# Project-MONAI/MONAI

Hardware: AMD Instinct MI355X
Metric: voxels/s sliding-window 3D seg (512^3 vol, 96^3 win, ov 0.5) at 1/8 GPU (higher is better)
Workload: dtype f32; 1 GPU; BasicUNet 5-class seed 1, 512^3 CT phantom in HBM, 96^3 win ov 0.5 gaussian, sw_batch 4 (engine: <= 64 windows per launch); parallelism=1 GPU

## Files before the change

### include/monai_amd.h

```cpp
#ifndef MONAI_AMD_H
#define MONAI_AMD_H

#include <stddef.h>
#include <stdint.h>

#ifdef __cplusplus
extern "C" {
#endif

#define MH_OK 0
#define MH_ERR_ARG (-1)
#define MH_ERR_LAUNCH (-2)
#define MH_ERR_UNSUPPORTED (-3)

typedef struct mh_tensor5 {
    float* data;
    int64_t n_stride;
    const float* nrm;
    int64_t nrm_n_stride;
    int32_t N, C, D, H, W;
} mh_tensor5;

int mh_version(void);
const char* mh_last_error(void);



int mh_window_extract_f32(const float* vol, int C, int D, int H, int W, const int32_t* sz, int nz,
                          const int32_t* sy, int ny, const int32_t* sx, int nx, int w0, int nwin, int rd, int rh,
                          int rw, float* out, void* stream);

int mh_sw_blend_f32(const float* logits, int64_t window_stride, const float* imp, float* out, int K, int D, int H, int W,
                    int rd, int rh, int rw, const int32_t* sz, int nz, const int32_t* sy, int ny, const int32_t* sx,
                    int nx, int premultiplied, void* stream);

int mh_sw_blend_buffered_f32(const float* logits, int64_t window_stride, const float* imp, float* out, int K, int D, int H, int W, int rd, int rh, int rw,
                             const int32_t* sz, int nz, const int32_t* sy, int ny, const int32_t* sx, int nx, int buffer_axis, int buffer_steps, int premultiplied, void* stream);

int mh_sw_mosaic_class_counts(int n, int log2m, int32_t* counts5);
int mh_sw_blend_mosaic_f32(const float* logits, const int64_t* class_base, int log2m_z, int log2m_y, int log2m_x, const float* imp, int imp_factored, float* out, int K,
                           int D, int H, int W, int rd, int rh, int rw, const int32_t* sz, int nz, const int32_t* sy, int ny, const int32_t* sx, int nx,
                           void* stream);

int mh_sw_blend_argmax_f32(const float* logits, int64_t window_stride, const float* imp, void* labels, int labels_u8, int K, int D,
                           int H, int W, int rd, int rh, int rw, const int32_t* sz, int nz, const int32_t* sy, int ny,
                           const int32_t* sx, int nx, int premultiplied, void* stream);

int mh_patch_accumulate_f32(float* values, uint8_t* counts, const float* patch, int NC, int D, int H, int W, int pd, int ph,
                            int pw, int z0, int y0, int x0, void* stream);
int mh_patch_accumulate_batch_f32(float* values, uint8_t* counts, const float* patches, int npatch, const int32_t* loc, int NC, int D, int H, int W,
                                  int pd, int ph, int pw, void* stream);
int mh_avg_finalize_f32(float* values, const uint8_t* counts, int64_t n, void* stream);


#define MH_ALGO_AUTO 0
#define MH_ALGO_DIRECT 1
#define MH_ALGO_WINO2D 2
#define MH_ALGO_H2 3
#define MH_ALGO_FP32 4
int mh_conv3d_k3_select(int algo, int input_bounded, int Cin, int Cout, int D, int H, int W);
int mh_conv3d_k3_num_configs(void);
int mh_conv3d_k3_h2_config(void);
int mh_conv3d_k3_h2c_config(void);
int mh_conv3d_k3_c1_config(void);
int mh_conv3d_k3_h2v_config(void);
int mh_conv3d_k3_h2w_config(void);
int mh_conv3d_k3_h2w_fits(int D, int H, int W);
int mh_conv3d_k3_accepts(int cfg, int Cin, int Cout);
int64_t mh_conv3d_k3_packed_floats(int cfg, int Cin, int Cout);
int mh_conv3d_k3_pack_f32(int cfg, const float* w, int Cin, int Cout, float* packed, void* stream);
int mh_conv3d_k3_stat_tiles(int cfg, int D, int H, int W);
int mh_conv3d_k3_f32(int cfg, const mh_tensor5* in, const float* packed_w, const float* bias,
                     const mh_tensor5* out, float* stats, void* stream);
int mh_conv3d_k3_pool_accepts(int cfg, int Cin, int Cout, int D, int H, int W);
int mh_conv3d_k3_pool_f32(int cfg, const mh_tensor5* in, const float* packed_w, const float* bias, const mh_tensor5* out, float* stats, float* pool_max, float* pool_min,
                          int64_t pool_n_stride, void* stream);
int mh_pool_select_f32(float* pool_max, const float* pool_min, const float* nrm, int64_t nrm_n_stride, int N, int C, int64_t n_stride, int64_t vol, void* stream);
int mh_conv3d_k3_accumulate_f32(int cfg, const mh_tensor5* in, const float* packed_w, const float* bias, const mh_tensor5* out, float* stats, void* stream);

int mh_instnorm_stat_tiles(int D, int H, int W);
int mh_instnorm_stats_f32(const mh_tensor5* x, float* stats, void* stream);
int mh_instnorm_finalize_f32(const float* stats, int tiles, int N, int C, const float* gamma, const float* beta,
                             float eps, float slope, float* nrm, int64_t nrm_n_stride, void* stream);
int mh_groupnorm_finalize_f32(const float* stats, int tiles, int N, int C, int groups, const float* gamma, const float* beta, float eps,
                              float slope, float* nrm, int64_t nrm_n_stride, void* stream);

int mh_nrm_identity_f32(float* nrm, int N, int C, int64_t nrm_n_stride, void* stream);

int mh_maxpool2_f32(const mh_tensor5* in, const mh_tensor5* out, void* stream);

int mh_deconv_k2s2_f32(const mh_tensor5* in, const float* w, const float* bias, const mh_tensor5* out,
                       void* stream);

int mh_deconv_k2s2_h2_accepts(int Cin, int Cout, int D, int H, int W);
int64_t mh_deconv_k2s2_h2_packed_floats(int Cin, int Cout);
int mh_deconv_k2s2_h2_pack_f32(const float* w, int Cin, int Cout, float* packed, void* stream);
int mh_deconv_k2s2_h2_f32(const mh_tensor5* in, const float* packed, const float* bias, const mh_tensor5* out, void* stream);

int mh_upconv_k4s2_accepts(int Cin, int Cout, int Dl, int Hl, int Wl);
int64_t mh_upconv_k4s2_packed_floats(int Cin, int Cout);
int mh_upconv_k4s2_pack_f32(const float* w4, int Cin, int Cout, float* packed, void* stream);
int mh_upconv_k4s2_stat_tiles(int Dl, int Hl, int Wl);
int mh_upconv_k4s2_f32(const mh_tensor5* low, const float* packed, const float* bias_table, const mh_tensor5* out, int accumulate, float* stats, void* stream);

int mh_conv3d_k3s2_accepts(int Cin, int Cout, int D, int H, int W);
int64_t mh_conv3d_k3s2_packed_floats(int Cin, int Cout);
int64_t mh_conv3d_k3s2_workspace_floats(int N, int Cin, int D, int H, int W);
int mh_conv3d_k3s2_stat_tiles(int D, int H, int W);
int mh_conv3d_k3s2_pack_f32(const float* w, int Cin, int Cout, float* packed, void* stream);
int mh_conv3d_k3s2_f32(const mh_tensor5* in, const float* packed, const float* bias, const mh_tensor5* out, float* workspace, float* stats, int fused, void* stream);

int mh_conv1x1_f32(const mh_tensor5* in, const float* w, const float* bias, const mh_tensor5* out,
                   void* stream);
int mh_conv1x1_stat_tiles(int D, int H, int W);
int mh_conv1x1_stats_f32(const mh_tensor5* in, const float* w, const float* bias, const mh_tensor5* out, float* stats, void* stream);

int mh_conv1x1_h2_accepts(int Cin, int Cout, int D, int H, int W);
int64_t mh_conv1x1_h2_packed_floats(int Cin, int Cout);
int mh_conv1x1_h2_pack_f32(const float* w, int Cout, int Cin, float* packed, void* stream);
int mh_conv1x1_h2_f32(const mh_tensor5* in, const float* packed, const float* bias, const mh_tensor5* out, float* stats, void* stream);

int mh_conv1x1_windows_f32(const mh_tensor5* in, const float* w, const float* bias, float* base, int Cout, const int64_t* place, void* stream);


int mh_add_act_f32(const mh_tensor5* a, const mh_tensor5* b, float slope, const mh_tensor5* out, void* stream);

int mh_conv1x1_sum2_accepts(int Cout, int D, int H, int W);
int mh_conv1x1_sum2_f32(const mh_tensor5* a, const mh_tensor5* b, float slope, const float* w, const float* bias, const mh_tensor5* out, void* stream);

int mh_pad_replicate_f32(const mh_tensor5* in, const mh_tensor5* out, void* stream);

int mh_pixelshuffle_f32(const mh_tensor5* in, const mh_tensor5* out, int fz, int pad_pool, void* stream);

int mh_attention_f32(const float* qkv, float* out, int B, int S, int heads, int head_dim, float scale, void* stream);

int mh_window_attention_f32(const float* qkv, const float* bias_t, const float* mask, float* out, int BW, int nW, int S, int heads,
                            int head_dim, float scale, int exact_fp32, void* stream);

int mh_window_attention_rel_accepts(int S, int head_dim, int table_rows);
int mh_window_attention_rel_f32(const float* qkv, const float* rel_table, int table_rows, const int32_t* coord, int coord_off, const int32_t* region,
                                float* out, int BW, int nW, int S, int heads, int head_dim, float scale, void* stream);

int64_t mh_linear_packed_floats(int N, int K);
int mh_linear_pack_f32(const float* w, int N, int K, float* packed, void* stream);
int mh_linear_f32(const float* x, const float* packed_w, const float* bias, const float* residual, float* y, int64_t M, int N, int K, int act,
                  void* stream);
int mh_linear_tile_f32(const float* x, const float* packed_w, const float* bias, const float* residual, float* y, int64_t M, int N, int K, int act,
                       int tile, void* stream);

int mh_layernorm_f32(const float* x, const float* gamma, const float* beta, float eps, float* y, int64_t M, int K, void* stream);

int mh_layernorm_gather_accepts(int K);
int mh_layernorm_gather_f32(const float* x, const float* gamma, const float* beta, float eps, float* y, int64_t M_out, int K, const int32_t* src_row, void* stream);
int mh_linear_scatter_f32(const float* x, const float* packed_w, const float* bias, const float* residual, float* y, int64_t M, int N, int K, int act,
                          const int32_t* dst_row, void* stream);


int mh_conv3d_k3_strided_f32(const mh_tensor5* in, const float* packed_w, const float* bias, const mh_tensor5* out,
                             int stride, void* stream);
int mh_conv3d_k3_strided3_f32(const mh_tensor5* in, const float* packed_w, const float* bias, const mh_tensor5* out, int sz, int sy, int sx,
                              void* stream);
int mh_deconv_ks_f32(const mh_tensor5* in, const float* w, const float* bias, const mh_tensor5* out, int fz, int fy, int fx, void* stream);

int mh_deconv_k3_f32(const mh_tensor5* in, const float* w, const float* bias, const mh_tensor5* out, int stride,
                     void* stream);


int64_t mh_affine_resample_workspace_bytes(int Do, int Ho, int Wo);
int mh_affine_resample_f32(const float* src, int NC, int Di, int Hi, int Wi, float* dst, int Do, int Ho, int Wo,
                           const double* m, int mode, int pad, int align_corners, int compute_f64, void* workspace,
                           void* stream);

int mh_grid_resample_f32(const float* src, int NC, int Di, int Hi, int Wi, const void* coords, int coords_f64,
                         const double* scale3, const double* offset3, float* dst, int Do, int Ho, int Wo, int mode,
                         int pad, int align_corners, int compute_f64, void* stream);

int mh_grid_pull(const void* src, const void* grid, void* out, int is_f64, int B, int C, int X, int Y, int Z, int Xo,
                 int Yo, int Zo, const int32_t* bound3, const int32_t* interp3, int extrapolate, void* stream);

int mh_pushpull(const void* source, const void* grid, const void* target, void* out, void* grad, int is_f64, int ndim, int B,
                int C, int X, int Y, int Z, int Xo, int Yo, int Zo, const int32_t* bound3, const int32_t* interp3,
                int extrapolate, int do_pull, int do_push, int do_count, int do_grad, int do_sgrad, int target_k, void* stream);


int mh_pointwise_f32(int op, const float* src, float* dst, int64_t n, float param, void* stream);
int mh_channel_reduce_f32(int op, const float* src, float* dst, int C, int64_t n, void* stream);
int mh_onehot_f32(const float* labels, float* dst, int K, int64_t n, void* stream);


int mh_scale_intensity_range_f32(const float* src, float* dst, int64_t n, float a_min, float a_div, int rescale, float b_scale, float b_min,
                                 int clip_lo, float lo, int clip_hi, float hi, void* stream);
int mh_foreground_bbox_workspace_ints(int D, int H);
int mh_foreground_bbox_f32(const float* src, int C, int D, int H, int W, int32_t* workspace, int32_t* box6, void* stream);
int mh_crop_pad_f32(const float* src, float* dst, int C, int D, int H, int W, int Do, int Ho, int Wo, int sz, int sy, int sx, float value,
                    void* stream);

int64_t mh_normalize_stats_workspace_doubles(int C, int64_t n);
int mh_normalize_stats_f32(const float* src, int C, int64_t n, int nonzero, double* workspace, float* subdiv, void* stream);
int mh_normalize_apply_f32(const float* src, float* dst, int C, int64_t n, int nonzero, const float* subdiv, void* stream);
int64_t mh_minmax_workspace_floats(int C, int64_t n);
int mh_minmax_f32(const float* src, int C, int64_t n, float* workspace, float* table, void* stream);
int mh_minmax_scale_f32(const float* src, float* dst, int C, int64_t n, const float* table, int rescale, float b_scale, float b_min,
                        int flat_has_mul, float flat_mul, void* stream);
int mh_flip_permute_f32(const float* src, float* dst, int C, const int32_t* in_size3, const int32_t* perm3, const int32_t* flip3, void* stream);


int mh_separable_filter3d_f32(const float* src, float* dst, int NC, int D, int H, int W, const float* kz, int kz_n,
                              const float* ky, int ky_n, const float* kx, int kx_n, void* stream);

#ifdef __cplusplus
}
#endif
#endif
```

### monai_amd/_lib.py

```python

from __future__ import annotations

import ctypes as C
import os
from typing import Optional, Sequence

import torch

from ._fallback import UnsupportedOnDevice

_HERE = os.path.dirname(os.path.abspath(__file__))
LIB_PATH = os.environ.get("MONAI_AMD_LIB") or os.path.join(_HERE, "csrc", "libmonai_amd.so")


class MhTensor5(C.Structure):

    _fields_ = [
        ("data", C.c_void_p),
        ("n_stride", C.c_int64),
        ("nrm", C.c_void_p),
        ("nrm_n_stride", C.c_int64),
        ("N", C.c_int32),
        ("C", C.c_int32),
        ("D", C.c_int32),
        ("H", C.c_int32),
        ("W", C.c_int32),
    ]


_I, _L, _P, _F = C.c_int, C.c_int64, C.c_void_p, C.c_float
_T = C.POINTER(MhTensor5)
_IA = C.POINTER(C.c_int32)

SIGNATURES = {
    "mh_version": (_I, []),
    "mh_last_error": (C.c_char_p, []),
    "mh_window_extract_f32": (_I, [_P, _I, _I, _I, _I, _IA, _I, _IA, _I, _IA, _I, _I, _I, _I, _I, _I, _P, _P]),
    "mh_patch_accumulate_f32": (_I, [_P, _P, _P] + [_I] * 10 + [_P]),
    "mh_patch_accumulate_batch_f32": (_I, [_P, _P, _P, _I, _IA] + [_I] * 7 + [_P]),
    "mh_avg_finalize_f32": (_I, [_P, _P, C.c_int64, _P]),
    "mh_pointwise_f32": (_I, [_I, _P, _P, _L, _F, _P]),
    "mh_channel_reduce_f32": (_I, [_I, _P, _P, _I, _L, _P]),
    "mh_onehot_f32": (_I, [_P, _P, _I, _L, _P]),
    "mh_scale_intensity_range_f32": (_I, [_P, _P, _L, _F, _F, _I, _F, _F, _I, _F, _I, _F, _P]),
    "mh_foreground_bbox_workspace_ints": (_I, [_I, _I]),
    "mh_foreground_bbox_f32": (_I, [_P, _I, _I, _I, _I, _P, _P, _P]),
    "mh_crop_pad_f32": (_I, [_P, _P] + [_I] * 10 + [_F, _P]),
    "mh_sw_blend_f32": (_I, [_P, _L, _P, _P, _I, _I, _I, _I, _I, _I, _I, _IA, _I, _IA, _I, _IA, _I, _I, _P]),
    "mh_sw_blend_buffered_f32": (_I, [_P, _L, _P, _P, _I, _I, _I, _I, _I, _I, _I, _IA, _I, _IA, _I, _IA, _I, _I, _I, _I, _P]),
    "mh_sw_mosaic_class_counts": (_I, [_I, _I, _IA]),
    "mh_sw_blend_mosaic_f32": (_I, [_P, C.POINTER(C.c_int64), _I, _I, _I, _P, _I, _P, _I, _I, _I, _I, _I, _I, _I, _IA, _I, _IA, _I, _IA, _I, _P]),
    "mh_sw_blend_argmax_f32": (_I, [_P, _L, _P, _P, _I, _I, _I, _I, _I, _I, _I, _I, _IA, _I, _IA, _I, _IA, _I, _I, _P]),
    "mh_conv3d_k3_select": (_I, [_I, _I, _I, _I, _I, _I, _I]),
    "mh_conv3d_k3_h2_config": (_I, []),
    "mh_conv3d_k3_h2c_config": (_I, []),
    "mh_conv3d_k3_c1_config": (_I, []),
    "mh_conv3d_k3_h2v_config": (_I, []),
    "mh_conv3d_k3_h2w_config": (_I, []),
    "mh_conv3d_k3_h2w_fits": (_I, [_I, _I, _I]),
    "mh_conv3d_k3_num_configs": (_I, []),
    "mh_conv3d_k3_accepts": (_I, [_I, _I, _I]),
    "mh_conv3d_k3_packed_floats": (_L, [_I, _I, _I]),
    "mh_conv3d_k3_pack_f32": (_I, [_I, _P, _I, _I, _P, _P]),
    "mh_conv3d_k3_stat_tiles": (_I, [_I, _I, _I, _I]),
    "mh_conv3d_k3_f32": (_I, [_I, _T, _P, _P, _T, _P, _P]),
    "mh_conv3d_k3_accumulate_f32": (_I, [_I, _T, _P, _P, _T, _P, _P]),
    "mh_conv3d_k3_pool_accepts": (_I, [_I, _I, _I, _I, _I, _I]),
    "mh_conv3d_k3_pool_f32": (_I, [_I, _T, _P, _P, _T, _P, _P, _P, _L, _P]),
    "mh_pool_select_f32": (_I, [_P, _P, _P, _L, _I, _I, _L, _L, _P]),
    "mh_instnorm_stat_tiles": (_I, [_I, _I, _I]),
    "mh_instnorm_stats_f32": (_I, [_T, _P, _P]),
    "mh_instnorm_finalize_f32": (_I, [_P, _I, _I, _I, _P, _P, _F, _F, _P, _L, _P]),
    "mh_groupnorm_finalize_f32": (_I, [_P, _I, _I, _I, _I, _P, _P, _F, _F, _P, _L, _P]),
    "mh_flip_permute_f32": (_I, [_P, _P, _I, _IA, _IA, _IA, _P]),
    "mh_normalize_stats_workspace_doubles": (_L, [_I, _L]),
    "mh_normalize_stats_f32": (_I, [_P, _I, _L, _I, _P, _P, _P]),
    "mh_normalize_apply_f32": (_I, [_P, _P, _I, _L, _I, _P, _P]),
    "mh_minmax_workspace_floats": (_L, [_I, _L]),
    "mh_minmax_f32": (_I, [_P, _I, _L, _P, _P, _P]),
    "mh_minmax_scale_f32": (_I, [_P, _P, _I, _L, _P, _I, _F, _F, _I, _F, _P]),
    "mh_nrm_identity_f32": (_I, [_P, _I, _I, _L, _P]),
    "mh_maxpool2_f32": (_I, [_T, _T, _P]),
    "mh_deconv_k2s2_f32": (_I, [_T, _P, _P, _T, _P]),
    "mh_upconv_k4s2_accepts": (_I, [_I, _I, _I, _I, _I]),
    "mh_upconv_k4s2_packed_floats": (_L, [_I, _I]),
    "mh_upconv_k4s2_pack_f32": (_I, [_P, _I, _I, _P, _P]),
    "mh_upconv_k4s2_stat_tiles": (_I, [_I, _I, _I]),
    "mh_upconv_k4s2_f32": (_I, [_T, _P, _P, _T, _I, _P, _P]),
    "mh_deconv_k2s2_h2_accepts": (_I, [_I, _I, _I, _I, _I]),
    "mh_deconv_k2s2_h2_packed_floats": (_L, [_I, _I]),
    "mh_deconv_k2s2_h2_pack_f32": (_I, [_P, _I, _I, _P, _P]),
    "mh_deconv_k2s2_h2_f32": (_I, [_T, _P, _P, _T, _P]),
    "mh_conv3d_k3s2_accepts": (_I, [_I, _I, _I, _I, _I]),
    "mh_conv3d_k3s2_packed_floats": (_L, [_I, _I]),
    "mh_conv3d_k3s2_workspace_floats": (_L, [_I, _I, _I, _I, _I]),
    "mh_conv3d_k3s2_stat_tiles": (_I, [_I, _I, _I]),
    "mh_conv3d_k3s2_pack_f32": (_I, [_P, _I, _I, _P, _P]),
    "mh_conv3d_k3s2_f32": (_I, [_T, _P, _P, _T, _P, _P, _I, _P]),
    "mh_conv1x1_f32": (_I, [_T, _P, _P, _T, _P]),
    "mh_conv1x1_stat_tiles": (_I, [_I, _I, _I]),
    "mh_conv1x1_stats_f32": (_I, [_T, _P, _P, _T, _P, _P]),
    "mh_conv1x1_h2_accepts": (_I, [_I, _I, _I, _I, _I]),
    "mh_conv1x1_h2_packed_floats": (_L, [_I, _I]),
    "mh_conv1x1_h2_pack_f32": (_I, [_P, _I, _I, _P, _P]),
    "mh_conv1x1_h2_f32": (_I, [_T, _P, _P, _T, _P, _P]),
    "mh_conv1x1_sum2_accepts": (_I, [_I, _I, _I, _I]),
    "mh_conv1x1_sum2_f32": (_I, [_T, _T, _F, _P, _P, _T, _P]),
    "mh_conv1x1_windows_f32": (_I, [_T, _P, _P, _P, _I, C.POINTER(C.c_int64), _P]),
    "mh_conv3d_k3_strided_f32": (_I, [_T, _P, _P, _T, _I, _P]),
    "mh_conv3d_k3_strided3_f32": (_I, [_T, _P, _P, _T, _I, _I, _I, _P]),
    "mh_deconv_ks_f32": (_I, [_T, _P, _P, _T, _I, _I, _I, _P]),
    "mh_deconv_k3_f32": (_I, [_T, _P, _P, _T, _I, _P]),
    "mh_add_act_f32": (_I, [_T, _T, _F, _T, _P]),
    "mh_pad_replicate_f32": (_I, [_T, _T, _P]),
    "mh_pixelshuffle_f32": (_I, [_T, _T, _I, _I, _P]),
    "mh_attention_f32": (_I, [_P, _P, _I, _I, _I, _I, _F, _P]),
    "mh_window_attention_f32": (_I, [_P, _P, _P, _P, _I, _I, _I, _I, _I, _F, _I, _P]),
    "mh_window_attention_rel_accepts": (_I, [_I, _I, _I]),
    "mh_window_attention_rel_f32": (_I, [_P, _P, _I, _P, _I, _P, _P, _I, _I, _I, _I, _I, _F, _P]),
    "mh_linear_packed_floats": (_L, [_I, _I]),
    "mh_linear_pack_f32": (_I, [_P, _I, _I, _P, _P]),
    "mh_linear_f32": (_I, [_P, _P, _P, _P, _P, _L, _I, _I, _I, _P]),
    "mh_linear_tile_f32": (_I, [_P, _P, _P, _P, _P, _L, _I, _I, _I, _I, _P]),
    "mh_layernorm_f32": (_I, [_P, _P, _P, _F, _P, _L, _I, _P]),
    "mh_layernorm_gather_accepts": (_I, [_I]),
    "mh_layernorm_gather_f32": (_I, [_P, _P, _P, _F, _P, _L, _I, _P, _P]),
    "mh_linear_scatter_f32": (_I, [_P, _P, _P, _P, _P, _L, _I, _I, _I, _P, _P]),
    "mh_affine_resample_workspace_bytes": (_L, [_I, _I, _I]),
    "mh_affine_resample_f32": (_I, [_P, _I, _I, _I, _I, _P, _I, _I, _I, C.POINTER(C.c_double), _I, _I, _I, _I, _P, _P]),
    "mh_separable_filter3d_f32": (_I, [_P, _P, _I, _I, _I, _I, C.POINTER(C.c_float), _I, C.POINTER(C.c_float), _I, C.POINTER(C.c_float), _I, _P]),
    "mh_grid_pull": (_I, [_P, _P, _P, _I, _I, _I, _I, _I, _I, _I, _I, _I, _IA, _IA, _I, _P]),
    "mh_pushpull": (_I, [_P, _P, _P, _P, _P] + [_I] * 10 + [_IA, _IA] + [_I] * 7 + [_P]),
    "mh_grid_resample_f32": (_I, [_P, _I, _I, _I, _I, _P, _I, C.POINTER(C.c_double), C.POINTER(C.c_double), _P, _I, _I, _I, _I, _I, _I, _I, _P]),
}


class KernelRejected(RuntimeError):
    """An entry point declined a VALID call it has no kernel for (MH_ERR_UNSUPPORTED: a size / shape rule) without launching: callers with an alternative
    path catch THIS, not RuntimeError.  Bad arguments (MH_ERR_ARG: null pointers, mismatched shapes, misalignment -- caller bugs), launch failures and HIP
    errors stay plain RuntimeErrors and must surface."""


class Library:

    def __init__(self, path: str):
        if not os.path.exists(path):
            raise RuntimeError(
                f"monai_amd: HIP extension not built ({path} missing). Run `python -m monai_amd.build` "
                "(hipcc --offload-arch=gfx950); there is no CPU fallback."
            )
        self.path = path
        self._dll = C.CDLL(path)
        for name, (res, args) in SIGNATURES.items():
            fn = getattr(self._dll, name)
            fn.restype, fn.argtypes = res, args
            setattr(self, "_" + name, fn)

    def last_error(self) -> str:
        return self._mh_last_error().decode("utf-8", "replace")

    def check(self, rc: int) -> None:
        if rc == -3:
            raise KernelRejected(f"monai_amd: {self.last_error()} (code {rc})")
        if rc != 0:
            raise RuntimeError(f"monai_amd: {self.last_error()} (code {rc})")

    def call(self, name: str, *args) -> None:
        self.check(getattr(self, "_" + name)(*args))

    def query(self, name: str, *args) -> int:
        rc = getattr(self, "_" + name)(*args)
        if rc < 0:
            raise RuntimeError(f"monai_amd: {self.last_error()} (code {rc})")
        return int(rc)


_LIB: Optional[Library] = None


def lib() -> Library:
    global _LIB
    if _LIB is None:
        _LIB = Library(LIB_PATH)
    return _LIB


def require_device(*tensors: torch.Tensor, dtypes=(torch.float32,)) -> None:
    for t in tensors:
        if t is None:
            continue
        if not t.is_cuda:
            raise UnsupportedOnDevice(
                "monai_amd: this path runs only on an MI355X (ROCm) device tensor; got a CPU tensor. "
                "There is no CPU fallback in the product path."
            )
        if t.dtype not in dtypes:
            raise UnsupportedOnDevice(f"monai_amd: dtype {t.dtype} is not accepted on this path (expected one of {dtypes})")


def stream_ptr(t: torch.Tensor) -> C.c_void_p:
    if t.is_cuda:
        return C.c_void_p(torch.cuda.current_stream(t.device).cuda_stream)
    return C.c_void_p(0)


def ptr(t: Optional[torch.Tensor]) -> C.c_void_p:
    return C.c_void_p(0 if t is None else t.data_ptr())


def int_array(values: Sequence[int]):
    return (C.c_int32 * len(values))(*[int(v) for v in values])


def tensor5(t: torch.Tensor, nrm: Optional[torch.Tensor] = None) -> MhTensor5:
    if t.dim() != 5:
        raise RuntimeError(f"monai_amd: expected a 5-D NCDHW tensor, got shape {tuple(t.shape)}")
    n, c, d, h, w = t.shape
    st = t.stride()
    if st[4] != 1 or st[3] != w or st[2] != h * w or st[1] != d * h * w:
# ... 12 lines not shown
```

### monai_amd/config.py

```python
import os

HAS_EXT = True
USE_COMPILED = HAS_EXT and os.getenv("BUILD_MONAI", "0") == "1"


CONV_ALGOS = {"auto": 0, "direct": 1, "wino2d": 2, "h2": 3, "fp32": 4}
CONV_ALGO = None


def conv_algo() -> int:
    name = CONV_ALGO if CONV_ALGO is not None else os.environ.get("MONAI_AMD_CONV_ALGO", "auto")
    try:
        return CONV_ALGOS[str(name).lower()]
    except KeyError:
        raise ValueError(f"monai_amd: unknown convolution family {name!r} (one of {sorted(CONV_ALGOS)})") from None


class conv_algo_scope:

    def __init__(self, name: str):
        if str(name).lower() not in CONV_ALGOS:
            raise ValueError(f"monai_amd: unknown convolution family {name!r} (one of {sorted(CONV_ALGOS)})")
        self.name = str(name).lower()

    def __enter__(self):
        global CONV_ALGO
        self._saved, CONV_ALGO = CONV_ALGO, self.name
        return self

    def __exit__(self, *exc):
        global CONV_ALGO
        CONV_ALGO = self._saved
        return False


UPCAT_FUSED = None


def upcat_fused() -> bool:
    v = UPCAT_FUSED if UPCAT_FUSED is not None else os.environ.get("MONAI_AMD_UPCAT_FUSED", "1")
    return str(v).lower() not in ("0", "false", "off", "no")


UPCAT_ORDER = None


def upcat_order() -> str:
    v = str(UPCAT_ORDER if UPCAT_ORDER is not None else os.environ.get("MONAI_AMD_UPCAT_ORDER", "conv_first")).lower()
    if v not in ("conv_first", "term_first"):
        raise ValueError(f"monai_amd: unknown UpCat order {v!r} (conv_first or term_first)")
    return v


CONV_HALVES = None


def conv_halves() -> bool:
    v = CONV_HALVES if CONV_HALVES is not None else os.environ.get("MONAI_AMD_CONV_HALVES", "1")
    return str(v).lower() not in ("0", "false", "off", "no")


RESIDUAL_ACC = None


def residual_accumulate() -> bool:
    v = RESIDUAL_ACC if RESIDUAL_ACC is not None else os.environ.get("MONAI_AMD_RESIDUAL_ACC", "1")
    return str(v).lower() not in ("0", "false", "off", "no")


POOL_FUSED = None


def pool_fused() -> bool:
    v = POOL_FUSED if POOL_FUSED is not None else os.environ.get("MONAI_AMD_POOL_FUSED", "1")
    return str(v).lower() not in ("0", "false", "off", "no")


STRIDED_H2 = None


def strided_h2() -> bool:
    v = STRIDED_H2 if STRIDED_H2 is not None else os.environ.get("MONAI_AMD_STRIDED_H2", "1")
    return str(v).lower() not in ("0", "false", "off", "no") and conv_algo() in (CONV_ALGOS["auto"], CONV_ALGOS["h2"])


STRIDED_H2_FUSED = None


def strided_h2_fused() -> str:
    v = str(STRIDED_H2_FUSED if STRIDED_H2_FUSED is not None else os.environ.get("MONAI_AMD_STRIDED_H2_FUSED", "auto")).lower()
    return "0" if v in ("0", "false", "off", "no") else ("1" if v in ("1", "true", "on", "yes") else "auto")


SMALL_VOLUME_H2 = None


def small_volume_h2() -> bool:
    v = SMALL_VOLUME_H2 if SMALL_VOLUME_H2 is not None else os.environ.get("MONAI_AMD_SMALL_VOLUME_H2", "1")
    return str(v).lower() not in ("0", "false", "off", "no")


DECONV_H2 = None


def deconv_h2() -> bool:
    v = DECONV_H2 if DECONV_H2 is not None else os.environ.get("MONAI_AMD_DECONV_H2", "1")
    return str(v).lower() not in ("0", "false", "off", "no") and conv_algo() in (CONV_ALGOS["auto"], CONV_ALGOS["h2"])


SWIN_FUSED_MOVES = None


def swin_fused_moves() -> bool:
    v = SWIN_FUSED_MOVES if SWIN_FUSED_MOVES is not None else os.environ.get("MONAI_AMD_SWIN_FUSED_MOVES", "1")
    return str(v).lower() not in ("0", "false", "off", "no")


SWIN_REL_ATTENTION = None


def swin_rel_attention() -> bool:
    v = SWIN_REL_ATTENTION if SWIN_REL_ATTENTION is not None else os.environ.get("MONAI_AMD_SWIN_REL_ATTENTION", "1")
    return str(v).lower() not in ("0", "false", "off", "no")
```

### monai_amd/csrc/capi.hip

```cpp
#include <hip/hip_runtime.h>

#include <stdarg.h>
#include <stdio.h>
#include <stdlib.h>
#include <string.h>

#include "kernels/common.h"
#include "kernels/attention.h"
#include "kernels/conv3d_mfma.h"
#include "kernels/conv3d_wino2p.h"
#include "kernels/conv3d_h2.h"
#include "kernels/conv3d_wino_h2.h"
#include "kernels/upconv_h2.h"
#include "kernels/conv3d_s2_h2.h"
#include "kernels/deconv_h2.h"
#include "kernels/conv3d_vol_h2.h"
#include "kernels/conv3d_c1.h"
#include "kernels/dense.h"
#include "kernels/gaussian.h"
#include "kernels/grid_pull.h"
#include "kernels/pushpull.h"
#include "kernels/post.h"
#include "kernels/preproc.h"
#include "kernels/nn_simple.h"
// ... 433 lines not shown
static inline int hw_blocks(int D, int H, int W) { return hw_regions(H, W) * cdiv(D, hw_zchunk(D, H, W)); }

int mh_conv3d_k3_num_configs(void) { return MH_CFG_WINO2D; }
int mh_conv3d_k3_h2_config(void) { return MH_CFG_H2; }
int mh_conv3d_k3_h2c_config(void) { return MH_CFG_H2C; }
int mh_conv3d_k3_c1_config(void) { return MH_CFG_C1; }
int mh_conv3d_k3_h2v_config(void) { return MH_CFG_H2V; }
int mh_conv3d_k3_h2w_config(void) { return MH_CFG_H2W; }
int mh_conv3d_k3_h2w_fits(int D, int H, int W) { return hw_fits(D, H, W) ? 1 : 0; }

int mh_conv3d_k3_pool_accepts(int cfg, int Cin, int Cout, int D, int H, int W) {
    if (cfg == MH_CFG_H2W) return Cin == HWG_CIN && Cout >= HWG_CN && Cout % HWG_CN == 0 && D % 2 == 0 && hw_fits(D, H, W);
    if (cfg != MH_CFG_H2 || D < 2 || H < 2 || W < 2 || D % 2 || H % 2 || W % 4) return 0;
    if (!(Cin >= H2_KC && Cin % H2_KC == 0 && Cin <= H2_NRM_MAX && Cout >= H2_CN && Cout % (H2_CN / 2) == 0) || !h2_fits(D, H, W)) return 0;
    return !h2_wide(H, W) && h2_zchunk(D, H, W) % 2 == 0;
}
int mh_conv3d_k3_accepts(int cfg, int Cin, int Cout) {
    if (cfg == 0) return 1;
    if (cfg == MH_CFG_WINO2D) return Cin >= 8 && Cin % 8 == 0 && Cout >= W2_CN && Cout % W2_CN == 0;
    if (cfg == MH_CFG_H2) return Cin >= H2_KC && Cin % H2_KC == 0 && Cin <= H2_NRM_MAX && Cout >= H2_CN && Cout % (H2_CN / 2) == 0;
    if (cfg == MH_CFG_H2C) return Cin >= H2_KC && Cin % H2_KC == 0 && Cin <= H2_NRM_MAX && Cout >= 16 && Cout % 16 == 0;
    if (cfg == MH_CFG_C1) return Cin == 1 && Cout >= 8 && Cout % 8 == 0;
    if (cfg == MH_CFG_H2V) return Cin >= 16 && Cin % 16 == 0 && Cin <= HV_CIN_MAX && Cout >= 32 && Cout % 32 == 0;
    if (cfg == MH_CFG_H2W) return Cin == HWG_CIN && Cout >= HWG_CN && Cout % HWG_CN == 0;
    if (cfg < 0 || cfg > MH_NUM_CFG) return 0;
    return Cout >= 1 && cin_padded(cfg, Cin) <= Cfg1::NRM_MAX;
}

int mh_conv3d_k3_select(int algo, int input_bounded, int Cin, int Cout, int D, int H, int W) {
    if (Cin < 1 || Cout < 1 || D < 1 || H < 1 || W < 1) return fail(MH_ERR_ARG, "conv3d_k3_select: bad argument");
    if (algo < MH_ALGO_AUTO || algo > MH_ALGO_FP32) return fail(MH_ERR_ARG, "conv3d_k3_select: unknown algorithm family %d", algo);
    int best = 0;
    double best_score = 0.0;
    for (int c = 1; c <= MH_NUM_CFG; ++c) {
        const CfgInfo& k = kCfg[c];
        if (!mh_conv3d_k3_accepts(c, Cin, Cout)) continue;
        const double util = (double)D * H * W / ((double)cdiv(D, k.tz) * k.tz * cdiv(H, k.ty) * k.ty * cdiv(W, k.tx) * k.tx);
        const double cpad = ((double)Cin / cin_padded(c, Cin)) * ((double)Cout / cout_padded(c, Cout));
        const double score = util * cpad * (1.0 + 0.02 * (k.cn / 32)) * kPref[c];
        if (score > best_score) { best_score = score; best = c; }
    }
    if (mh_conv3d_k3_accepts(MH_CFG_WINO2D, Cin, Cout) && H % 2 == 0 && W % 8 == 0) {
        const bool big = H % W2_B == 0 && W % W2_B == 0 && D >= 48 && H >= 48 && W >= 48;
        if (algo == MH_ALGO_WINO2D || ((algo == MH_ALGO_AUTO || algo == MH_ALGO_FP32) && big)) best = MH_CFG_WINO2D;
    }
    if ((algo == MH_ALGO_AUTO || algo == MH_ALGO_H2) && input_bounded && mh_conv3d_k3_accepts(MH_CFG_H2, Cin, Cout) && W % 4 == 0 && H >= 8 && W >= 8 && h2_fits(D, H, W))
        best = MH_CFG_H2;
    if ((algo == MH_ALGO_AUTO || algo == MH_ALGO_H2) && input_bounded && Cout == 16 && mh_conv3d_k3_accepts(MH_CFG_H2C, Cin, Cout) && W % 4 == 0 && H >= 8 && W >= 8 && h2_fits(D, H, W)
        && knob_int("MONAI_AMD_H2C", 1) != 0)
        best = MH_CFG_H2C;
    if ((algo == MH_ALGO_AUTO || algo == MH_ALGO_H2) && input_bounded && best != MH_CFG_H2 && best != MH_CFG_H2C && mh_conv3d_k3_accepts(MH_CFG_H2V, Cin, Cout) && hv_fits(D, H, W))
        best = MH_CFG_H2V;
    if (algo == MH_ALGO_AUTO && best == MH_CFG_H2 && mh_conv3d_k3_accepts(MH_CFG_H2W, Cin, Cout) && hw_fits(D, H, W) && D >= 24 && knob_int("MONAI_AMD_H2W", MH_H2W_DEFAULT) != 0)
        best = MH_CFG_H2W;
    if (algo != MH_ALGO_DIRECT && algo != MH_ALGO_WINO2D && mh_conv3d_k3_accepts(MH_CFG_C1, Cin, Cout) && W % 4 == 0 && knob_int("MONAI_AMD_C1", 1) != 0)
        best = MH_CFG_C1;
    return best;
}

int64_t mh_conv3d_k3_packed_floats(int cfg, int Cin, int Cout) {
    if (cfg == MH_CFG_WINO2D) return (int64_t)(Cin / W2_KC) * (Cout / W2_CN) * W2_UBUF;
    if (cfg == MH_CFG_H2) return (int64_t)(Cin / H2_KC) * cdiv(Cout, H2_CN) * H2_WB * 4 + H2_TAIL;
    if (cfg == MH_CFG_H2C) return (int64_t)(Cin / H2_KC) * (Cout / 16) * H2_WB * 4 + H2_TAIL;
    if (cfg == MH_CFG_C1) return (int64_t)27 * Cout;
    if (cfg == MH_CFG_H2V) return (int64_t)Cout * Cin * 27 + H2_TAIL;
    if (cfg == MH_CFG_H2W) return (int64_t)(Cout / HWG_CN) * HWG_WAVES * HWG_OPS * 64 * 4 + H2_TAIL;
    if (cfg < 0 || cfg > MH_NUM_CFG) return fail(MH_ERR_ARG, "conv3d_k3: unknown configuration %d", cfg);
    return (int64_t)cin_padded(cfg, Cin) * cout_padded(cfg, Cout) * 27;
}

int mh_conv3d_k3_pack_f32(int cfg, const float* w, int Cin, int Cout, float* packed, void* stream) {
    if (cfg == MH_CFG_WINO2D) {
        if (!w || !packed || !mh_conv3d_k3_accepts(cfg, Cin, Cout)) return fail(MH_ERR_ARG, "conv3d_k3_pack: in-plane Winograd needs Cin %% 8 == 0, Cout %% 16 == 0");
        if (hipMemsetAsync(packed, 0, sizeof(float) * (size_t)mh_conv3d_k3_packed_floats(cfg, Cin, Cout), (hipStream_t)stream) != hipSuccess)
            return fail(MH_ERR_LAUNCH, "conv3d_k3_pack: memset failed");
        hipLaunchKernelGGL(conv3d_k3_wino2d_pack_kernel, dim3(blocks_for((long long)Cin * Cout)), dim3(256), 0, (hipStream_t)stream, w, Cin, Cout, packed);
        return launched("conv3d_k3_wino2d_pack");
    }
    if (cfg == MH_CFG_H2C) {
        if (!w || !packed || !mh_conv3d_k3_accepts(cfg, Cin, Cout)) return fail(MH_ERR_ARG, "conv3d_k3_pack: the 16-couts fp16 split kernel needs Cin %% 16 == 0, Cout %% 16 == 0");
        const int64_t slab_floats = mh_conv3d_k3_packed_floats(cfg, Cin, Cout) - H2_TAIL;
        float* tail = packed + slab_floats;
        if (hipMemsetAsync(packed, 0, sizeof(float) * (size_t)slab_floats, (hipStream_t)stream) != hipSuccess)
            return fail(MH_ERR_LAUNCH, "conv3d_k3_pack: memset failed");
        hipLaunchKernelGGL(conv3d_k3_h2_scale_kernel, dim3(1), dim3(1024), 0, (hipStream_t)stream, w, (long long)Cin * Cout * 27, tail);
        hipLaunchKernelGGL(conv3d_k3_h2c_pack_kernel, dim3(blocks_for((long long)Cin * Cout)), dim3(256), 0, (hipStream_t)stream, w, Cin, Cout,
                           reinterpret_cast<_Float16*>(packed), tail);
        return launched("conv3d_k3_h2c_pack");
    }
    if (cfg == MH_CFG_H2) {
        if (!w || !packed || !mh_conv3d_k3_accepts(cfg, Cin, Cout)) return fail(MH_ERR_ARG, "conv3d_k3_pack: the fp16 split kernel needs Cin %% 16 == 0, Cout %% 16 == 0, Cout >= 32");
        const int64_t slab_floats = mh_conv3d_k3_packed_floats(cfg, Cin, Cout) - H2_TAIL;
        float* tail = packed + slab_floats;
        if (hipMemsetAsync(packed, 0, sizeof(float) * (size_t)slab_floats, (hipStream_t)stream) != hipSuccess)
            return fail(MH_ERR_LAUNCH, "conv3d_k3_pack: memset failed");
        hipLaunchKernelGGL(conv3d_k3_h2_scale_kernel, dim3(1), dim3(1024), 0, (hipStream_t)stream, w, (long long)Cin * Cout * 27, tail);
        hipLaunchKernelGGL(conv3d_k3_h2_pack_kernel, dim3(blocks_for((long long)Cin * Cout)), dim3(256), 0, (hipStream_t)stream, w, Cin, Cout,
                           reinterpret_cast<_Float16*>(packed), tail);
        return launched("conv3d_k3_h2_pack");
    }
    if (cfg == MH_CFG_H2W) {
        if (!w || !packed || !mh_conv3d_k3_accepts(cfg, Cin, Cout)) return fail(MH_ERR_ARG, "conv3d_k3_pack: the Winograd split kernel needs Cin == 32, Cout %% 32 == 0");
        float* tail = packed + (mh_conv3d_k3_packed_floats(cfg, Cin, Cout) - H2_TAIL);
        hipLaunchKernelGGL(conv3d_k3_h2_scale_kernel, dim3(1), dim3(1024), 0, (hipStream_t)stream, w, (long long)Cin * Cout * 27, tail);
        hipLaunchKernelGGL(conv3d_k3_h2w_scale_fix_kernel, dim3(1), dim3(64), 0, (hipStream_t)stream, tail);
        hipLaunchKernelGGL(conv3d_k3_h2w_pack_kernel, dim3(blocks_for((long long)Cin * Cout)), dim3(256), 0, (hipStream_t)stream, w, Cin, Cout,
                           reinterpret_cast<_Float16*>(packed), tail);
        return launched("conv3d_k3_h2w_pack");
    }
    if (cfg == MH_CFG_H2V) {
        if (!w || !packed || !mh_conv3d_k3_accepts(cfg, Cin, Cout)) return fail(MH_ERR_ARG, "conv3d_k3_pack: the small-volume split kernel needs Cin %% 16 == 0 (<= 768), Cout %% 32 == 0");
        float* tail = packed + (mh_conv3d_k3_packed_floats(cfg, Cin, Cout) - H2_TAIL);
        hipLaunchKernelGGL(conv3d_k3_h2_scale_kernel, dim3(1), dim3(1024), 0, (hipStream_t)stream, w, (long long)Cin * Cout * 27, tail);
        hipLaunchKernelGGL(conv3d_k3_vol_h2_pack_kernel, dim3(blocks_for((long long)Cin * Cout)), dim3(256), 0, (hipStream_t)stream, w, Cin, Cout, Cout % 64 == 0 ? 2 : 1,
                           reinterpret_cast<_Float16*>(packed), tail);
        return launched("conv3d_k3_vol_h2_pack");
    }
    if (cfg == MH_CFG_C1) {
        if (!w || !packed || !mh_conv3d_k3_accepts(cfg, Cin, Cout)) return fail(MH_ERR_ARG, "conv3d_k3_pack: the one-channel kernel needs Cin == 1, Cout %% 8 == 0");
        hipLaunchKernelGGL(conv3d_k3_pack_kernel, dim3(blocks_for(27LL * Cout)), dim3(256), 0, (hipStream_t)stream, w, 1, 1, Cout, Cout, Cout, packed);
        return launched("conv3d_k3_pack");
    }
    if (cfg < 0 || cfg > MH_NUM_CFG || !w || !packed) return fail(MH_ERR_ARG, "conv3d_k3_pack: bad argument");
    const int cn = cfg == 0 ? Cout : kCfg[cfg].cn;
    const int cinp = cin_padded(cfg, Cin), coutp = cout_padded(cfg, Cout);
    hipLaunchKernelGGL(conv3d_k3_pack_kernel, dim3(blocks_for((long long)cinp * coutp * 27)), dim3(256), 0, (hipStream_t)stream, w,
                       Cin, cinp, Cout, coutp, cn, packed);
    return launched("conv3d_k3_pack");
}

int mh_conv3d_k3_stat_tiles(int cfg, int D, int H, int W) {
    if (cfg == MH_CFG_WINO2D) return wino2d_blocks(D, H, W);
    if (cfg == MH_CFG_H2 || cfg == MH_CFG_H2C) return h2_blocks(D, H, W);
    if (cfg == MH_CFG_C1) return c1_blocks(D, H, W);
    if (cfg == MH_CFG_H2V) return 1;
    if (cfg == MH_CFG_H2W) return hw_fits(D, H, W) ? hw_blocks(D, H, W) : 0;
    if (cfg < 1 || cfg > MH_NUM_CFG) return 0;
    const CfgInfo& k = kCfg[cfg];
    return cdiv(W, k.tx) * cdiv(H, k.ty) * cdiv(D, k.tz);
}

template <class Cfg>
static void launch_mfma(const Tensor& in, const float* wp, const float* bias, const Tensor& out, float* stats, hipStream_t s) {
    const int tx = cdiv(out.W, Cfg::TX), ty = cdiv(out.H, Cfg::TY), tz = cdiv(out.D, Cfg::TZ);
    const dim3 grid((unsigned)(tx * ty * tz), (unsigned)cdiv(out.C, Cfg::CN), (unsigned)out.N);
    if (stats)
        hipLaunchKernelGGL((conv3d_k3_mfma_kernel<Cfg, true>), grid, dim3(256), 0, s, in, wp, bias, out, stats, tx, ty, tz);
    else
        hipLaunchKernelGGL((conv3d_k3_mfma_kernel<Cfg, false>), grid, dim3(256), 0, s, in, wp, bias, out, stats, tx, ty, tz);
}

struct PoolOut { float* mx; float* mn; long long n_stride; };
static int conv3d_k3_launch(int cfg, const mh_tensor5* in_, const float* packed_w, const float* bias, const mh_tensor5* out_, float* stats, void* stream, bool accumulate,
                            const PoolOut* pool = nullptr);
int mh_conv3d_k3_pool_accepts(int cfg, int Cin, int Cout, int D, int H, int W);
int mh_conv3d_k3_pool_f32(int cfg, const mh_tensor5* in_, const float* packed_w, const float* bias, const mh_tensor5* out_, float* stats, float* pool_max, float* pool_min,
                          int64_t pool_n_stride, void* stream) {
    if (!in_ || !out_ || !pool_max || !pool_min || !stats || !in_->nrm) return fail(MH_ERR_ARG, "conv3d_k3_pool: input records, statistics and both pooled tensors are required");
    if (!mh_conv3d_k3_pool_accepts(cfg, in_->C, out_->C, out_->D, out_->H, out_->W))
        return fail(MH_ERR_UNSUPPORTED, "conv3d_k3_pool: the pooling epilogue exists for the split-precision configuration on even extents with 16 x 16 regions");
    if (!aligned(pool_max, 8) || !aligned(pool_min, 8) || pool_n_stride % 2 || (long long)out_->C * (out_->D / 2) * (out_->H / 2) * (out_->W / 2) > pool_n_stride)
        return fail(MH_ERR_ARG, "conv3d_k3_pool: pooled tensors must be 8-byte aligned [N][>= C][D/2][H/2][W/2]");
    const PoolOut po{pool_max, pool_min, (long long)pool_n_stride};
    return conv3d_k3_launch(cfg, in_, packed_w, bias, out_, stats, stream, false, &po);
}
int mh_pool_select_f32(float* pool_max, const float* pool_min, const float* nrm, int64_t nrm_n_stride, int N, int C, int64_t n_stride, int64_t vol, void* stream) {
    if (!pool_max || !pool_min || !nrm || N < 1 || C < 1 || vol < 1) return fail(MH_ERR_ARG, "pool_select: bad argument");
    const unsigned nb = (unsigned)std::min<long long>(blocks_for(vol), 64);
    hipLaunchKernelGGL(pool_select_kernel, dim3(nb, (unsigned)C, (unsigned)N), dim3(256), 0, (hipStream_t)stream, pool_max, pool_min, nrm, (long long)nrm_n_stride, (long long)n_stride, (long long)vol);
    return launched("pool_select");
}
int mh_conv3d_k3_f32(int cfg, const mh_tensor5* in_, const float* packed_w, const float* bias, const mh_tensor5* out_,
                     float* stats, void* stream) {
    return conv3d_k3_launch(cfg, in_, packed_w, bias, out_, stats, stream, false);
}
int mh_conv3d_k3_accumulate_f32(int cfg, const mh_tensor5* in_, const float* packed_w, const float* bias, const mh_tensor5* out_,
                                float* stats, void* stream) {
    if ((cfg != MH_CFG_H2 && cfg != MH_CFG_H2C && cfg != MH_CFG_H2W) || !stats || !in_ || !in_->nrm)
        return fail(MH_ERR_UNSUPPORTED, "conv3d_k3_accumulate: the accumulating form exists for the split-precision configuration with input records and statistics");
    return conv3d_k3_launch(cfg, in_, packed_w, bias, out_, stats, stream, true);
}
static int conv3d_k3_launch(int cfg, const mh_tensor5* in_, const float* packed_w, const float* bias, const mh_tensor5* out_,
                            float* stats, void* stream, bool accumulate, const PoolOut* pool) {
    if (!dense_ok(in_) || !dense_ok(out_) || !packed_w) return fail(MH_ERR_ARG, "conv3d_k3: bad tensor");
    const Tensor in = from_c(*in_), out = from_c(*out_);
    if (in.N != out.N || in.D != out.D || in.H != out.H || in.W != out.W) return fail(MH_ERR_ARG, "conv3d_k3: shape mismatch");
    if (cfg < 0 || cfg > MH_CFG_LAST) return fail(MH_ERR_ARG, "conv3d_k3: unknown configuration %d", cfg);
    if (in.nrm && !aligned(in.nrm, 16)) return fail(MH_ERR_ARG, "conv3d_k3: nrm must be 16-byte aligned");
    hipStream_t s = (hipStream_t)stream;
    if (cfg == MH_CFG_C1) {
        if (!mh_conv3d_k3_accepts(cfg, in.C, out.C) || in.W % 4)
            return fail(MH_ERR_ARG, "conv3d_k3: the one-channel kernel needs Cin == 1, Cout %% 8 == 0, W %% 4 == 0 (got %d -> %d, %dx%dx%d)", in.C, out.C,
                        in.D, in.H, in.W);
        if (!aligned(out.data, 16) || out.n_stride % 4 || !aligned(in.data, 16) || in.n_stride % 4 || !aligned(packed_w, 4))
            return fail(MH_ERR_ARG, "conv3d_k3: the one-channel kernel needs 16-byte aligned input and output");
        const int txn = cdiv(out.W, C1_TX), tyn = cdiv(out.H, C1_TY), zc = c1_zchunk(out.D);
        constexpr int cot = 8;
        const dim3 grid((unsigned)(txn * tyn * cdiv(out.D, zc)), (unsigned)(out.C / cot), (unsigned)out.N);
        if (stats && in.nrm) hipLaunchKernelGGL((conv3d_k3_c1_kernel<cot, true, true>), grid, dim3(256), 0, s, in, packed_w, bias, out, stats, txn, tyn, zc);
        else if (stats) hipLaunchKernelGGL((conv3d_k3_c1_kernel<cot, true, false>), grid, dim3(256), 0, s, in, packed_w, bias, out, stats, txn, tyn, zc);
        else if (in.nrm) hipLaunchKernelGGL((conv3d_k3_c1_kernel<cot, false, true>), grid, dim3(256), 0, s, in, packed_w, bias, out, stats, txn, tyn, zc);
        else hipLaunchKernelGGL((conv3d_k3_c1_kernel<cot, false, false>), grid, dim3(256), 0, s, in, packed_w, bias, out, stats, txn, tyn, zc);
        return launched("conv3d_k3_c1");
    }
    if (cfg == MH_CFG_H2W) {
        if (!mh_conv3d_k3_accepts(cfg, in.C, out.C) || !hw_fits(in.D, in.H, in.W))
            return fail(MH_ERR_ARG, "conv3d_k3: the Winograd split kernel needs Cin == 32, Cout %% 32 == 0, H %% 4 == 0, W %% 16 == 0, D*H*W < 2^24 (got %d -> %d, %dx%dx%d)",
                        in.C, out.C, in.D, in.H, in.W);
        if (!in.nrm) return fail(MH_ERR_ARG, "conv3d_k3: the Winograd split kernel needs input records with magnitude bounds");
        if (!aligned(out.data, 16) || out.n_stride % 4 || !aligned(packed_w, 16)) return fail(MH_ERR_ARG, "conv3d_k3: the Winograd split kernel needs 16-byte aligned output and weights");
        if ((accumulate || pool) && !stats) return fail(MH_ERR_ARG, "conv3d_k3: the accumulating / pooling forms leave statistics");
        const int bxn = out.W / HWG_BX, byn = out.H / HWG_BY, zc = hw_zchunk(out.D, out.H, out.W);
        const unsigned nblk = (unsigned)(bxn * byn * cdiv(out.D, zc));
        const long long total = (long long)nblk * (out.C / HWG_CN) * out.N;
        if (total > 0x7fffffffLL) return fail(MH_ERR_UNSUPPORTED, "conv3d_k3: problem too large for one launch");
        const dim3 grid((unsigned)total);
        const uint4* wq = reinterpret_cast<const uint4*>(packed_w);
        const float* tail = packed_w + (mh_conv3d_k3_packed_floats(cfg, in.C, out.C) - H2_TAIL);
        if (pool) hipLaunchKernelGGL((conv3d_k3_h2w_kernel<true, false, true>), grid, dim3(64 * HWG_WAVES), 0, s, in, wq, tail, bias, out, stats, bxn, byn, zc, nblk, pool->mx, pool->mn, pool->n_stride);
        else if (accumulate) hipLaunchKernelGGL((conv3d_k3_h2w_kernel<true, true, false>), grid, dim3(64 * HWG_WAVES), 0, s, in, wq, tail, bias, out, stats, bxn, byn, zc, nblk, (float*)nullptr, (float*)nullptr, 0LL);
        else if (stats) hipLaunchKernelGGL((conv3d_k3_h2w_kernel<true, false, false>), grid, dim3(64 * HWG_WAVES), 0, s, in, wq, tail, bias, out, stats, bxn, byn, zc, nblk, (float*)nullptr, (float*)nullptr, 0LL);
        else hipLaunchKernelGGL((conv3d_k3_h2w_kernel<false, false, false>), grid, dim3(64 * HWG_WAVES), 0, s, in, wq, tail, bias, out, stats, bxn, byn, zc, nblk, (float*)nullptr, (float*)nullptr, 0LL);
        return launched("conv3d_k3_h2w");
    }
    if (cfg == MH_CFG_H2V) {
        if (accumulate || pool) return fail(MH_ERR_UNSUPPORTED, "conv3d_k3: the small-volume split kernel has no accumulating / pooling form");
        if (!mh_conv3d_k3_accepts(cfg, in.C, out.C) || !hv_fits(in.D, in.H, in.W))
            return fail(MH_ERR_ARG, "conv3d_k3: the small-volume split kernel needs Cin %% 16 == 0 (<= 768), Cout %% 32 == 0, 64 <= D*H*W <= 256, (D+2)(H+2)(W+2) <= 512 (got %d -> %d, %dx%dx%d)",
                        in.C, out.C, in.D, in.H, in.W);
        if (!in.nrm) return fail(MH_ERR_ARG, "conv3d_k3: the small-volume split kernel needs input records with magnitude bounds");
        if (!aligned(out.data, 16) || out.n_stride % 4 || !aligned(packed_w, 16)) return fail(MH_ERR_ARG, "conv3d_k3: the small-volume split kernel needs 16-byte aligned output and weights");
        const int ncgw = out.C % 64 == 0 ? 2 : 1;
        const long long total = (long long)(out.C / (32 * ncgw)) * out.N;
        if (total > 0x7fffffffLL) return fail(MH_ERR_UNSUPPORTED, "conv3d_k3: problem too large for one launch");
        const uint4* wq = reinterpret_cast<const uint4*>(packed_w);
        const float* tail = packed_w + (mh_conv3d_k3_packed_floats(cfg, in.C, out.C) - H2_TAIL);
        const dim3 grid((unsigned)total);
        if (ncgw == 2) {
            if (stats) hipLaunchKernelGGL((conv3d_k3_vol_h2_kernel<2, true>), grid, dim3(HV_NT), 0, s, in, wq, tail, bias, out, stats);
            else hipLaunchKernelGGL((conv3d_k3_vol_h2_kernel<2, false>), grid, dim3(HV_NT), 0, s, in, wq, tail, bias, out, stats);
        } else {
            if (stats) hipLaunchKernelGGL((conv3d_k3_vol_h2_kernel<1, true>), grid, dim3(HV_NT), 0, s, in, wq, tail, bias, out, stats);
            else hipLaunchKernelGGL((conv3d_k3_vol_h2_kernel<1, false>), grid, dim3(HV_NT), 0, s, in, wq, tail, bias, out, stats);
        }
        return launched("conv3d_k3_vol_h2");
    }
    if (cfg == MH_CFG_H2 || cfg == MH_CFG_H2C) {
        const bool c16 = cfg == MH_CFG_H2C;
        if (!mh_conv3d_k3_accepts(cfg, in.C, out.C) || in.W % 4)
            return fail(MH_ERR_ARG, "conv3d_k3: the fp16 split kernel needs Cin %% 16 == 0, Cout %% 16 == 0 (>= 32; any multiple of 16 in its 16-couts form), W %% 4 == 0 (got %d -> %d, %dx%dx%d)",
                        in.C, out.C, in.D, in.H, in.W);
        if (!aligned(out.data, 16) || out.n_stride % 4 || !aligned(packed_w, 16))
            return fail(MH_ERR_ARG, "conv3d_k3: the fp16 split kernel needs 16-byte aligned output and weights");
        if (!h2_fits(out.D, out.H, out.W))
            return fail(MH_ERR_UNSUPPORTED, "conv3d_k3: the fp16 split kernel addresses 32 output planes with 32-bit offsets (D*H*W < 2^24 voxels); mh_conv3d_k3_select does not return it beyond");
        const bool wide = h2_wide(out.H, out.W);
        const int bxn = wide ? cdiv(out.W, 32) : cdiv(out.W, H2_B), byn = wide ? cdiv(out.H, 8) : cdiv(out.H, H2_B), zc = h2_zchunk(out.D, out.H, out.W);
        const unsigned nblk = (unsigned)(bxn * byn * cdiv(out.D, zc));
        const long long total = (long long)nblk * (c16 ? out.C / 16 : cdiv(out.C, H2_CN)) * out.N;
        if (total > 0x7fffffffLL) return fail(MH_ERR_UNSUPPORTED, "conv3d_k3: problem too large for one launch");
        const dim3 grid((unsigned)total);
        const uint4* wq = reinterpret_cast<const uint4*>(packed_w);
        const float* tail = packed_w + (mh_conv3d_k3_packed_floats(cfg, in.C, out.C) - H2_TAIL);
#define MH_H2_LAUNCH(RES_, WIDE_, C16_)                                                                                                                  \
    {                                                                                                                                                \
        if (stats && in.nrm) hipLaunchKernelGGL((conv3d_k3_h2_kernel<true, true, RES_, WIDE_, C16_>), grid, dim3(512), 0, s, in, wq, tail, bias, out, stats, bxn, byn, zc, nblk, (float*)nullptr, (float*)nullptr, 0LL);   \
        else if (stats) hipLaunchKernelGGL((conv3d_k3_h2_kernel<true, false, RES_, WIDE_, C16_>), grid, dim3(512), 0, s, in, wq, tail, bias, out, stats, bxn, byn, zc, nblk, (float*)nullptr, (float*)nullptr, 0LL);       \
        else if (in.nrm) hipLaunchKernelGGL((conv3d_k3_h2_kernel<false, true, RES_, WIDE_, C16_>), grid, dim3(512), 0, s, in, wq, tail, bias, out, stats, bxn, byn, zc, nblk, (float*)nullptr, (float*)nullptr, 0LL);      \
        else hipLaunchKernelGGL((conv3d_k3_h2_kernel<false, false, RES_, WIDE_, C16_>), grid, dim3(512), 0, s, in, wq, tail, bias, out, stats, bxn, byn, zc, nblk, (float*)nullptr, (float*)nullptr, 0LL);                 \
    }
        if (pool) {
#define MH_H2_POOL(RES_) hipLaunchKernelGGL((conv3d_k3_h2_kernel<true, true, RES_, false, false, false, true>), grid, dim3(512), 0, s, in, wq, tail, bias, out, stats, bxn, byn, zc, nblk, pool->mx, pool->mn, pool->n_stride)
            if (in.C <= 2 * H2_KC) MH_H2_POOL(true); else MH_H2_POOL(false);
#undef MH_H2_POOL
            return launched("conv3d_k3_h2_pool");
        }
        if (accumulate) {
#define MH_H2_ACC(RES_, WIDE_, C16_) hipLaunchKernelGGL((conv3d_k3_h2_kernel<true, true, RES_, WIDE_, C16_, true>), grid, dim3(512), 0, s, in, wq, tail, bias, out, stats, bxn, byn, zc, nblk, (float*)nullptr, (float*)nullptr, 0LL)
            if (c16) {
                if (in.C <= 2 * H2_KC) { if (wide) MH_H2_ACC(true, true, true); else MH_H2_ACC(true, false, true); }
                else { if (wide) MH_H2_ACC(false, true, true); else MH_H2_ACC(false, false, true); }
            } else {
                if (in.C <= 2 * H2_KC) { if (wide) MH_H2_ACC(true, true, false); else MH_H2_ACC(true, false, false); }
                else { if (wide) MH_H2_ACC(false, true, false); else MH_H2_ACC(false, false, false); }
            }
#undef MH_H2_ACC
            return launched("conv3d_k3_h2_acc");
        }
        if (c16) {
            if (in.C <= 2 * H2_KC) { if (wide) MH_H2_LAUNCH(true, true, true) else MH_H2_LAUNCH(true, false, true) }
            else { if (wide) MH_H2_LAUNCH(false, true, true) else MH_H2_LAUNCH(false, false, true) }
        } else {
            if (in.C <= 2 * H2_KC) { if (wide) MH_H2_LAUNCH(true, true, false) else MH_H2_LAUNCH(true, false, false) }
            else { if (wide) MH_H2_LAUNCH(false, true, false) else MH_H2_LAUNCH(false, false, false) }
        }
#undef MH_H2_LAUNCH
        return launched(c16 ? "conv3d_k3_h2c" : "conv3d_k3_h2");
    }
    if (cfg == MH_CFG_WINO2D) {
        if (!mh_conv3d_k3_accepts(cfg, in.C, out.C) || in.H % 2 || in.W % 8)
            return fail(MH_ERR_ARG, "conv3d_k3: in-plane Winograd needs Cin %% 8 == 0, Cout %% 16 == 0, even H and W %% 8 == 0 (got %d -> %d, %dx%dx%d)",
                        in.C, out.C, in.D, in.H, in.W);
        if (!aligned(out.data, 16) || out.n_stride % 4 || !aligned(packed_w, 16))
            return fail(MH_ERR_ARG, "conv3d_k3: in-plane Winograd needs 16-byte aligned output and weights");
        const int bxn = cdiv(out.W, W2_B), byn = cdiv(out.H, W2_B), zc = wino2d_zchunk(out.D, out.H, out.W);
        const unsigned nblk = (unsigned)(bxn * byn * cdiv(out.D, zc));
        const long long total = (long long)nblk * (out.C / W2_CN) * out.N;
        if (total > 0x7fffffffLL) return fail(MH_ERR_UNSUPPORTED, "conv3d_k3: problem too large for one launch");
        const dim3 grid((unsigned)total);
        if (stats && in.nrm) hipLaunchKernelGGL((conv3d_k3_wino2p_kernel<true, true>), grid, dim3(512), 0, s, in, packed_w, bias, out, stats, bxn, byn, zc, nblk);
        else if (stats) hipLaunchKernelGGL((conv3d_k3_wino2p_kernel<true, false>), grid, dim3(512), 0, s, in, packed_w, bias, out, stats, bxn, byn, zc, nblk);
        else if (in.nrm) hipLaunchKernelGGL((conv3d_k3_wino2p_kernel<false, true>), grid, dim3(512), 0, s, in, packed_w, bias, out, stats, bxn, byn, zc, nblk);
        else hipLaunchKernelGGL((conv3d_k3_wino2p_kernel<false, false>), grid, dim3(512), 0, s, in, packed_w, bias, out, stats, bxn, byn, zc, nblk);
        return launched("conv3d_k3_wino2p");
    }
    if (cfg == 0) {
        if (stats) return fail(MH_ERR_ARG, "conv3d_k3: the direct kernel emits no statistics");
        constexpr int COT = 16;
        const dim3 grid(blocks_for((long long)out.D * out.H * out.W), (unsigned)cdiv(out.C, COT), (unsigned)out.N);
        hipLaunchKernelGGL((conv3d_k3_direct_kernel<COT>), grid, dim3(256), 0, s, in, packed_w, bias, out);
        return launched("conv3d_k3_direct");
    }
    const CfgInfo& k = kCfg[cfg];
    (void)k;
    if (!mh_conv3d_k3_accepts(cfg, in.C, out.C))
        return fail(MH_ERR_ARG, "conv3d_k3: configuration %d does not take Cin=%d Cout=%d", cfg, in.C, out.C);
    if (!aligned(packed_w, 16)) return fail(MH_ERR_ARG, "conv3d_k3: packed weights must be 16-byte aligned");
    switch (cfg) {
        case 1: launch_mfma<Cfg1>(in, packed_w, bias, out, stats, s); break;
        case 2: launch_mfma<Cfg2>(in, packed_w, bias, out, stats, s); break;
        case 3: launch_mfma<Cfg3>(in, packed_w, bias, out, stats, s); break;
        case 4: launch_mfma<Cfg4>(in, packed_w, bias, out, stats, s); break;
        case 5: launch_mfma<Cfg5>(in, packed_w, bias, out, stats, s); break;
        case 6: launch_mfma<Cfg6>(in, packed_w, bias, out, stats, s); break;
        case 7: launch_mfma<Cfg7>(in, packed_w, bias, out, stats, s); break;
        case 8: launch_mfma<Cfg8>(in, packed_w, bias, out, stats, s); break;
        case 9: launch_mfma<Cfg9>(in, packed_w, bias, out, stats, s); break;
        case 10: launch_mfma<Cfg10>(in, packed_w, bias, out, stats, s); break;
        case 11: launch_mfma<Cfg11>(in, packed_w, bias, out, stats, s); break;
        case 12: launch_mfma<Cfg12>(in, packed_w, bias, out, stats, s); break;
        case 13: launch_mfma<Cfg13>(in, packed_w, bias, out, stats, s); break;
        case 14: launch_mfma<Cfg14>(in, packed_w, bias, out, stats, s); break;
    }
    return launched("conv3d_k3_mfma");
}

int mh_instnorm_stat_tiles(int D, int H, int W) {
    return (int)(((long long)D * H * W + STAT_CHUNK - 1) / STAT_CHUNK);
}

int mh_instnorm_stats_f32(const mh_tensor5* x_, float* stats, void* stream) {
    if (!dense_ok(x_) || !stats) return fail(MH_ERR_ARG, "instnorm_stats: bad argument");
    const Tensor x = from_c(*x_);
    const int tiles = mh_instnorm_stat_tiles(x.D, x.H, x.W);
    hipLaunchKernelGGL(instnorm_stats_kernel, dim3((unsigned)tiles, (unsigned)x.C, (unsigned)x.N), dim3(256), 0,
                       (hipStream_t)stream, x, stats, tiles);
    return launched("instnorm_stats");
}

int mh_instnorm_finalize_f32(const float* stats, int tiles, int N, int C, const float* gamma, const float* beta, float eps,
                             float slope, float* nrm, int64_t nrm_n_stride, void* stream) {
    if (!stats || !nrm || tiles < 1 || N < 1 || C < 1 || nrm_n_stride < 4LL * C) return fail(MH_ERR_ARG, "instnorm_finalize: bad argument");
    hipLaunchKernelGGL(instnorm_finalize_kernel, dim3((unsigned)C, (unsigned)N), dim3(64), 0, (hipStream_t)stream, stats, tiles,
                       C, 1, gamma, beta, eps, slope, nrm, (long long)nrm_n_stride);
    return launched("instnorm_finalize");
}

int mh_groupnorm_finalize_f32(const float* stats, int tiles, int N, int C, int groups, const float* gamma, const float* beta, float eps,
                              float slope, float* nrm, int64_t nrm_n_stride, void* stream) {
    if (!stats || !nrm || tiles < 1 || N < 1 || C < 1 || groups < 1 || C % groups || nrm_n_stride < 4LL * C)
        return fail(MH_ERR_ARG, "groupnorm_finalize: bad argument (channels must be divisible by groups)");
    hipLaunchKernelGGL(instnorm_finalize_kernel, dim3((unsigned)groups, (unsigned)N), dim3(64), 0, (hipStream_t)stream, stats, tiles,
                       C, C / groups, gamma, beta, eps, slope, nrm, (long long)nrm_n_stride);
    return launched("groupnorm_finalize");
}
// ... 1153 lines not shown
```

### monai_amd/csrc/kernels/common.h

```cpp
#pragma once
#include <hip/hip_runtime.h>
#include <stdint.h>

#include "../../../include/monai_amd.h"

#ifdef MH_SIMT_EMULATOR
#define MH_OPAQUE(x) ((void)0)
#define MH_OPAQUE_S(x) ((void)0)
#else
#define MH_OPAQUE(x) asm volatile("" : "+v"(x))
#define MH_OPAQUE_S(x) asm volatile("" : "+s"(x))
#endif

typedef int mh_i32x4 __attribute__((ext_vector_type(4)));
#ifdef MH_SIMT_EMULATOR
#define MH_LDS_DMA_F32(BASE, VOFF, LDS_WAVE_BASE) ((void)((LDS_WAVE_BASE)[threadIdx.x & 63] = *reinterpret_cast<const float*>(reinterpret_cast<const char*>(BASE) + (VOFF))))
#define MH_VMCNT_BARRIER(N) __syncthreads()
#define MH_VMCNT_WAIT(N) ((void)0)
#else
#define MH_LDS_DMA_F32(BASE, VOFF, LDS_WAVE_BASE)                                                                                             \
    {                                                                                                                                         \
        const unsigned long long b_ = (unsigned long long)(BASE);       \
        const mh_i32x4 r_ = {__builtin_amdgcn_readfirstlane((int)(unsigned)b_), __builtin_amdgcn_readfirstlane((int)((unsigned)(b_ >> 32) & 0xffffu)), 0x7fffffff, 0x00020000}; \
         \
        const unsigned m_ = (unsigned)__builtin_amdgcn_readfirstlane((int)(unsigned)(unsigned long long)(LDS_WAVE_BASE)); \
        asm volatile("s_mov_b32 m0, %0\n\ts_nop 0\n\tbuffer_load_dword %1, %2, 0 offen lds" ::"s"(m_), "v"(VOFF), "s"(r_) : "memory", "m0"); \
    }
#define MH_VMCNT_IMM(N) (0x0f70 | ((N) & 15) | ((((N) >> 4) & 3) << 14))
#define MH_VMCNT_BARRIER(N) do { __builtin_amdgcn_s_waitcnt(MH_VMCNT_IMM(N)); __builtin_amdgcn_s_barrier(); } while (0)
#define MH_VMCNT_WAIT(N) __builtin_amdgcn_s_waitcnt(MH_VMCNT_IMM(N))
#endif

#define MH_STREAM_STORE4(ptr, val) __builtin_nontemporal_store((val), reinterpret_cast<mh::f32x4*>(ptr))

namespace mh {

typedef float f32x16 __attribute__((ext_vector_type(16)));
typedef float f32x4 __attribute__((ext_vector_type(4)));
typedef float f32x2 __attribute__((ext_vector_type(2)));
typedef _Float16 f16x8 __attribute__((ext_vector_type(8)));
typedef _Float16 f16x4 __attribute__((ext_vector_type(4)));
typedef _Float16 f16x2 __attribute__((ext_vector_type(2)));
typedef unsigned u32x4 __attribute__((ext_vector_type(4)));
typedef unsigned u32x2 __attribute__((ext_vector_type(2)));

struct Tensor {
    float* data;
    long long n_stride;
    const float* nrm;
    long long nrm_n_stride;
    int N, C, D, H, W;
};

__host__ __device__ inline Tensor from_c(const mh_tensor5& t) {
    Tensor r;
    r.data = t.data; r.n_stride = t.n_stride; r.nrm = t.nrm; r.nrm_n_stride = t.nrm_n_stride;
    r.N = t.N; r.C = t.C; r.D = t.D; r.H = t.H; r.W = t.W;
    return r;
}

__device__ __forceinline__ float act(float x, float alpha, float beta, float slope) {
    float y = fmaf(x, alpha, beta);
    return y > 0.0f ? y : y * slope;
}

__device__ __forceinline__ float4 load_nrm(const Tensor& t, int n, int c) {
    if (t.nrm == nullptr) return make_float4(1.0f, 0.0f, 1.0f, 0.0f);
    return *reinterpret_cast<const float4*>(t.nrm + (long long)n * t.nrm_n_stride + 4LL * c);
}

constexpr float MH_BOUND_FLOOR = 1.17549435e-38f;
__device__ __forceinline__ unsigned abs_bits(float v) { return __float_as_uint(v) & 0x7fffffffu; }
__device__ __forceinline__ unsigned wave_umax(unsigned m) {
#pragma unroll
    for (int o = 32; o > 0; o >>= 1) {
        const unsigned t = (unsigned)__shfl_xor((int)m, o);
        m = t > m ? t : m;
    }
    return m;
}
__device__ __forceinline__ void bound_commit(unsigned m, float* slot) {
    m = wave_umax(m);
    if ((threadIdx.x & 63) == 0 && m != 0u) atomicMax(reinterpret_cast<unsigned*>(slot), m);
}
__device__ __forceinline__ float* bound_slot(const Tensor& t, int n, int c) {
    return const_cast<float*>(t.nrm) + (long long)n * t.nrm_n_stride + 4LL * c + 3;
}

struct Stat {
    float n, mean, m2;
};
__device__ __forceinline__ Stat stat_merge(Stat a, Stat b) {
    Stat r;
    r.n = a.n + b.n;
    if (r.n <= 0.0f) { r.mean = 0.0f; r.m2 = 0.0f; return r; }
    const float d = b.mean - a.mean;
    const float f = b.n / r.n;
    r.mean = a.mean + d * f;
    r.m2 = a.m2 + b.m2 + d * d * a.n * f;
    return r;
}
__device__ __forceinline__ float lane_left(float edge, float v) {
    int r = __builtin_amdgcn_update_dpp(__builtin_bit_cast(int, edge), __builtin_bit_cast(int, v), 0x138, 0xf, 0xf, false);
    MH_OPAQUE(r);
    return __builtin_bit_cast(float, r);
}
__device__ __forceinline__ float lane_right(float edge, float v) {
    int r = __builtin_amdgcn_update_dpp(__builtin_bit_cast(int, edge), __builtin_bit_cast(int, v), 0x130, 0xf, 0xf, false);
    MH_OPAQUE(r);
    return __builtin_bit_cast(float, r);
}

__device__ __forceinline__ Stat stat_merge_nb(Stat a, Stat b) {
    Stat r;
    r.n = a.n + b.n;
    const bool e = r.n <= 0.0f;
    const float d = b.mean - a.mean;
    const float f = b.n / (e ? 1.0f : r.n);
    r.mean = e ? 0.0f : a.mean + d * f;
    r.m2 = e ? 0.0f : a.m2 + b.m2 + d * d * a.n * f;
    return r;
}

__device__ __forceinline__ unsigned xcd_remap(unsigned b, unsigned nb) {
    const unsigned q = nb / 8u, r = nb % 8u, x = b % 8u, i = b / 8u;
    return (x < r ? x * (q + 1u) : r * (q + 1u) + (x - r) * q) + i;
}

}
```

### monai_amd/csrc/kernels/conv3d_wino_h2.h

```cpp
#pragma once
#include "common.h"
#include "conv3d_h2.h"

namespace mh {

constexpr int HWG_BY = 4, HWG_BX = 16;
constexpr int HWG_RY = HWG_BY + 2, HWG_RX = HWG_BX + 2;
constexpr int HWG_NP = HWG_RY * HWG_RX;
constexpr int HWG_PB = 144;
constexpr int HWG_DB = (HWG_NP + 1) * HWG_PB;
constexpr int HWG_ZB = 32 * 1024;
constexpr int HWG_OPS = 24;
constexpr int HWG_CIN = 32, HWG_CN = 32;
constexpr int HWG_WAVES = 8;
constexpr unsigned HWG_DROP = 0x80000000u;

__device__ __forceinline__ void hw_split4(const f32x4 v, u32x2& hi, u32x2& lo) {
    _Float16 h_[4], l_[4];
#pragma unroll
    for (int i = 0; i < 4; ++i) {
        h_[i] = (_Float16)v[i];
        float r = v[i] - (float)h_[i];
        MH_OPAQUE(r);
        l_[i] = (_Float16)r;
    }
    const f16x2 h01 = {h_[0], h_[1]}, h23 = {h_[2], h_[3]}, l01 = {l_[0], l_[1]}, l23 = {l_[2], l_[3]};
    hi = u32x2{__builtin_bit_cast(unsigned, h01), __builtin_bit_cast(unsigned, h23)};
    lo = u32x2{__builtin_bit_cast(unsigned, l01), __builtin_bit_cast(unsigned, l23)};
}

__device__ __forceinline__ f32x4 hw_fma4(const f32x4 a, const float s, const f32x4 c) { return __builtin_elementwise_fma(a, f32x4{s, s, s, s}, c); }
__device__ __forceinline__ void hw_split4p(const f32x4 v, const float m1, u32x2& hi, u32x2& lo) {
#ifdef MH_SIMT_EMULATOR
    f16x2 h01, l01, h23, l23;
    h2_split_pair(v[0], v[1], m1, h01, l01);
    h2_split_pair(v[2], v[3], m1, h23, l23);
    hi = u32x2{__builtin_bit_cast(unsigned, h01), __builtin_bit_cast(unsigned, h23)};
    lo = u32x2{__builtin_bit_cast(unsigned, l01), __builtin_bit_cast(unsigned, l23)};
#else
    unsigned h0, h1, l0, l1;
    asm("v_cvt_pk_f16_f32 %0, %1, %2" : "=v"(h0) : "v"(v[0]), "v"(v[1]));
    asm("v_cvt_pk_f16_f32 %0, %1, %2" : "=v"(h1) : "v"(v[2]), "v"(v[3]));
    asm("v_fma_mixlo_f16 %0, %1, %2, %3 op_sel_hi:[1,0,0]" : "=v"(l0) : "v"(h0), "v"(m1), "v"(v[0]));
    asm("v_fma_mixlo_f16 %0, %1, %2, %3 op_sel_hi:[1,0,0]" : "=v"(l1) : "v"(h1), "v"(m1), "v"(v[2]));
    asm("v_fma_mixhi_f16 %0, %1, %2, %3 op_sel:[1,0,0] op_sel_hi:[1,0,0]" : "+v"(l0) : "v"(h0), "v"(m1), "v"(v[1]));
    asm("v_fma_mixhi_f16 %0, %1, %2, %3 op_sel:[1,0,0] op_sel_hi:[1,0,0]" : "+v"(l1) : "v"(h1), "v"(m1), "v"(v[3]));
    hi = u32x2{h0, h1};
    lo = u32x2{l0, l1};
#endif
}
__device__ __forceinline__ float hw_xchg32(const float x, const int hi) {
#ifdef MH_SIMT_EMULATOR
    (void)hi;
    return __shfl_xor(x, 32);
#else
    const auto r = __builtin_amdgcn_permlane32_swap(__builtin_bit_cast(unsigned, x), __builtin_bit_cast(unsigned, x), false, false);
    return __builtin_bit_cast(float, hi ? r[0] : r[1]);
#endif
}
#ifdef MH_SIMT_EMULATOR
#define MH_HW_KEEP_BRANCH ((void)0)
#else
#define MH_HW_KEEP_BRANCH asm volatile("" ::: "memory")
#endif

template <bool STATS, bool ACC = false, bool POOL = false>
__global__ void __launch_bounds__(512)
conv3d_k3_h2w_kernel(Tensor in, const uint4* __restrict__ wp, const float* __restrict__ wtail, const float* __restrict__ bias, Tensor out,
                     float* __restrict__ stats, int bxn, int byn, int zchunk, unsigned nblk, float* __restrict__ pmax, float* __restrict__ pmin,
                     long long pool_n_stride) {
    __shared__ __attribute__((aligned(16))) char smem[3 * HWG_DB + 2 * HWG_ZB];
    __shared__ unsigned bound_s[4];
    char* const ds = smem;
    char* const zs_ = smem + 3 * HWG_DB;
    const int tid = threadIdx.x, lane = tid & 63;
    const int wave = __builtin_amdgcn_readfirstlane(tid >> 6);
    const int wi = wave & 3, jp = wave >> 2;
    const int Cout = out.C, D = out.D, H = out.H, W = out.W;
    const long long HW = (long long)H * W, DHW = (long long)D * HW;

    const unsigned ncg = (unsigned)(Cout / HWG_CN);
    unsigned lid = xcd_remap(blockIdx.x, gridDim.x);
    const int cg = (int)(lid % ncg);
    lid /= ncg;
    const unsigned b = lid % nblk;
    const int n = (int)(lid / nblk);
    const int x0 = (int)(b % bxn) * HWG_BX, y0 = (int)((b / bxn) % byn) * HWG_BY;
    const int zs = (int)(b / (bxn * byn)) * zchunk, ze = min(zs + zchunk, D);
    const int p_first = max(zs - 1, 0), p_last = min(ze, D - 1);

    unsigned soff;
    int loff[2];
    {
        const int pr = min(lane, 53);
        const int ly = pr / 9;
        int lx = 2 * (pr - 9 * ly);
        const int gy = y0 + ly - 1;
        int gx = x0 + lx - 1;
        if (gx < 0) { gx += 1; lx += 1; }
        if (gx + 1 >= W) { gx -= 1; lx -= 1; }
        const bool ok = lane < 54 && gy >= 0 && gy < H;
        soff = ok ? 4u * (unsigned)(gy * W + gx) : 0u;
        loff[0] = (ok ? ly * HWG_RX + lx : HWG_NP) * HWG_PB;
        loff[1] = (ok ? ly * HWG_RX + lx + 1 : HWG_NP) * HWG_PB;
    }
    for (int i = tid; i < (3 * HWG_DB + 2 * HWG_ZB) / 16; i += 512) reinterpret_cast<uint4*>(smem)[i] = make_uint4(0u, 0u, 0u, 0u);
    f32x4 nra, nrb, nrs;
    {
        unsigned mb = 0u;
        if (lane < HWG_CIN) {
            const float4 a = *reinterpret_cast<const float4*>(in.nrm + (long long)n * in.nrm_n_stride + 4LL * lane);
            const unsigned bb = abs_bits(a.w);
            mb = bb == 0u ? 0x7fc00000u : bb;
        }
        mb = wave_umax(mb);
        if (tid == 0) bound_s[0] = mb;
    }
    __syncthreads();
    int e_in = 0;
    bool poisoned = false;
    {
        const unsigned mb = bound_s[0];
        poisoned = mb >= 0x7f800000u;
        e_in = poisoned ? 0 : min(max(13 - ((int)(mb >> 23) - 126), -100), 100);
        const float p_ = __uint_as_float((unsigned)(e_in + 127) << 23);
#pragma unroll
        for (int i = 0; i < 4; ++i) {
            const float4 a = *reinterpret_cast<const float4*>(in.nrm + (long long)n * in.nrm_n_stride + 4LL * (4 * wave + i));
            nra[i] = a.x * p_; nrb[i] = a.y * p_; nrs[i] = a.z;
        }
    }
    f32x4 nrk;
#pragma unroll
    for (int i = 0; i < 4; ++i) nrk[i] = nrs[i] <= 1.0f ? __builtin_inff() : -__builtin_inff();
    const auto xrs = __builtin_amdgcn_make_buffer_rsrc(const_cast<float*>(in.data + (long long)n * in.n_stride + (long long)(4 * wave) * DHW), 0, 0x7fffffff, 0x00020000);
    const unsigned hw4 = (unsigned)(HW * 4);
    unsigned voff = soff + (unsigned)p_first * hw4;
    const unsigned cso1 = (unsigned)(DHW * 4), cso2 = 2u * cso1, cso3 = 3u * cso1;
    f32x2 xin[4];
#define MH_HW_LDX                                                                                     \
    {                                                                                                 \
        xin[0] = __builtin_bit_cast(f32x2, __builtin_amdgcn_raw_buffer_load_b64(xrs, voff, 0u, 0));   \
        xin[1] = __builtin_bit_cast(f32x2, __builtin_amdgcn_raw_buffer_load_b64(xrs, voff, cso1, 0)); \
        xin[2] = __builtin_bit_cast(f32x2, __builtin_amdgcn_raw_buffer_load_b64(xrs, voff, cso2, 0)); \
        xin[3] = __builtin_bit_cast(f32x2, __builtin_amdgcn_raw_buffer_load_b64(xrs, voff, cso3, 0)); \
    }
#define MH_HW_CONV(DBO)                                                                               \
    {                                                                                                 \
        char* const db_ = ds + (DBO) + 16 * wave;                                                     \
        _Pragma("unroll") for (int j = 0; j < 2; ++j) {                                               \
            f32x4 y_;                                                                                 \
            const f32x4 t_ = __builtin_elementwise_fma(f32x4{xin[0][j], xin[1][j], xin[2][j], xin[3][j]}, nra, nrb), u_ = t_ * nrs; \
            _Pragma("unroll") for (int i = 0; i < 4; ++i) y_[i] = __builtin_amdgcn_fmed3f(t_[i], u_[i], nrk[i]);       \
            *reinterpret_cast<f32x4*>(db_ + loff[j]) = y_;                                            \
        }                                                                                             \
    }
    int staged = p_first;
#define MH_HW_ADV { voff += staged < p_last ? hw4 : 0u; staged += 1; }

    u32x4 wu[HWG_OPS];
    {
        const u32x4* wg = reinterpret_cast<const u32x4*>(wp) + ((long long)(cg * 8 + wave) * HWG_OPS) * 64 + lane;
#pragma unroll
        for (int r = 0; r < HWG_OPS; ++r) wu[r] = wg[r * 64];
    }
#define MH_HW_U(SL, T, CB, PC) __builtin_bit_cast(f16x8, wu[(((SL) * 3 + (T)) * 2 + (CB)) * 2 + (PC)])

    const int rho = lane & 15, kg = lane >> 4;
    const int tty = (rho >= 4 && rho < 12) ? 1 : 0, ttx = rho < 4 ? rho : rho < 12 ? rho - 4 : rho - 8;
    const int ra = wi == 0 ? 0 : wi == 2 ? 2 : 1, rb = wi == 0 ? 2 : wi == 1 ? 2 : wi == 2 ? 1 : 3;
    const float sgn = wi == 1 ? 1.0f : -1.0f;
    const float fsg = jp ? -1.0f : 1.0f;
    const float m1 = h2_minus_one();
    const int ab0 = ((2 * tty + ra) * HWG_RX + 2 * ttx + jp) * HWG_PB + kg * 16;
    const int ab1 = ((2 * tty + rb) * HWG_RX + 2 * ttx + jp) * HWG_PB + kg * 16;

    f32x4 acc[3][2][2];
#pragma unroll
    for (int s = 0; s < 3; ++s)
#pragma unroll
        for (int j = 0; j < 2; ++j)
#pragma unroll
            for (int c = 0; c < 2; ++c) acc[s][j][c] = f32x4{0.0f, 0.0f, 0.0f, 0.0f};

    const int fcb = wave >> 2, frp = (wave >> 1) & 1, fh = wave & 1;
    const int il = 32 * fh + (lane & 31), fa = lane >> 5;
    const int g4 = il >> 4;
    const int fty = (g4 == 1 || g4 == 2) ? 1 : 0, ftx = (g4 >= 2 ? 4 : 0) + 2 * frp;
    const int co_l = fcb * 16 + (il & 15), co = cg * HWG_CN + co_l;
    const float bco = bias ? bias[co] : 0.0f;
    const float fs2 = fa ? -1.0f : 1.0f;
    const int zwr = wave * 4096 + lane * 16;
    const int zrd = fa * 4096 + fcb * 2048 + il * 16 + frp * 8;
    float inv_a, inv_b;
    {
        const int t_ = -((int)((__float_as_uint(wtail[1]) >> 23) & 0xffu) - 127) - e_in;
        const int t1_ = t_ / 2, t2_ = t_ - t1_;
        inv_a = poisoned ? __uint_as_float(0x7fc00000u) : __uint_as_float((unsigned)(t1_ + 127) << 23);
        inv_b = __uint_as_float((unsigned)(t2_ + 127) << 23);
    }
    const auto orsrc = __builtin_amdgcn_make_buffer_rsrc(out.data + (long long)n * out.n_stride + (long long)(cg * HWG_CN) * DHW, 0, (int)(HWG_CN * DHW * 4), 0x00020000);
    const unsigned ooff = 4u * (unsigned)((long long)co_l * DHW + (long long)(y0 + 2 * fty + fa) * W + x0 + 2 * ftx);
    float pivot = 0.0f;
    bool have_c = false;
    f32x4 s1 = {0.0f, 0.0f, 0.0f, 0.0f}, s2 = s1;
    const long long PHW = (long long)(H / 2) * (W / 2), PDHW = (long long)(D / 2) * PHW;
    const auto prs = __builtin_amdgcn_make_buffer_rsrc(POOL ? (fa ? pmin : pmax) + (long long)n * pool_n_stride + (long long)(cg * HWG_CN) * PDHW : out.data, 0, POOL ? (int)(HWG_CN * PDHW * 4) : 0, 0x00020000);
    const unsigned poff = 4u * (unsigned)((long long)co_l * PDHW + (long long)((y0 >> 1) + fty) * (W / 2) + (x0 >> 1) + ftx);
    const float pk_ = fa ? -__builtin_inff() : __builtin_inff();
    f32x2 hm = {0.0f, 0.0f};
    f32x4 pv = {0.0f, 0.0f, 0.0f, 0.0f};

    u32x4 ah[2], al[2];
#define MH_HW_XFORM(DBO)                                                                              \
    {                                                                                                 \
        const char* const db_ = ds + (DBO);                                                           \
        _Pragma("unroll") for (int h = 0; h < 2; ++h) {                                               \
            f32x4 r_[3];                                                                              \
            _Pragma("unroll") for (int bq = 0; bq < 3; ++bq) {                                        \
                const f32x4 u_ = *reinterpret_cast<const f32x4*>(db_ + ab0 + bq * HWG_PB + h * 64);   \
                const f32x4 v_ = *reinterpret_cast<const f32x4*>(db_ + ab1 + bq * HWG_PB + h * 64);   \
                r_[bq] = hw_fma4(v_, sgn, u_);                                                        \
            }                                                                                         \
            const f32x4 e_ = hw_fma4(r_[2], m1, r_[0]);                                               \
            f32x4 f_;                                                                                 \
            if (jp) { f_ = hw_fma4(r_[0], m1, r_[1]); MH_HW_KEEP_BRANCH; } else f_ = r_[1] + r_[2];   \
            u32x2 hh_, ll_;                                                                           \
            hw_split4p(e_, m1, hh_, ll_); ah[0][2 * h] = hh_[0]; ah[0][2 * h + 1] = hh_[1]; al[0][2 * h] = ll_[0]; al[0][2 * h + 1] = ll_[1]; \
            hw_split4p(f_, m1, hh_, ll_); ah[1][2 * h] = hh_[0]; ah[1][2 * h + 1] = hh_[1]; al[1][2 * h] = ll_[0]; al[1][2 * h + 1] = ll_[1]; \
        }                                                                                             \
    }
#define MH_HW_MM(S, SL, CB, A, B, FRESH)                                                              \
    acc[S][SL][CB] = __builtin_amdgcn_mfma_f32_16x16x32_f16(__builtin_bit_cast(f16x8, A), B, (FRESH) ? f32x4{0.0f, 0.0f, 0.0f, 0.0f} : acc[S][SL][CB], 0, 0, 0);
#define MH_HW_MMS(S0, S1, S2)                                                                         \
    _Pragma("unroll") for (int sl = 0; sl < 2; ++sl)                                                  \
        _Pragma("unroll") for (int cb = 0; cb < 2; ++cb) {                                            \
            MH_HW_MM(S0, sl, cb, ah[sl], MH_HW_U(sl, 0, cb, 0), true)  MH_HW_MM(S1, sl, cb, ah[sl], MH_HW_U(sl, 1, cb, 0), false) MH_HW_MM(S2, sl, cb, ah[sl], MH_HW_U(sl, 2, cb, 0), false) \
            MH_HW_MM(S0, sl, cb, al[sl], MH_HW_U(sl, 0, cb, 0), false) MH_HW_MM(S1, sl, cb, al[sl], MH_HW_U(sl, 1, cb, 0), false) MH_HW_MM(S2, sl, cb, al[sl], MH_HW_U(sl, 2, cb, 0), false) \
            MH_HW_MM(S0, sl, cb, ah[sl], MH_HW_U(sl, 0, cb, 1), false) MH_HW_MM(S1, sl, cb, ah[sl], MH_HW_U(sl, 1, cb, 1), false) MH_HW_MM(S2, sl, cb, ah[sl], MH_HW_U(sl, 2, cb, 1), false) \
        }
#define MH_HW_SKIP(S0)                                                                                \
    { _Pragma("unroll") for (int sl = 0; sl < 2; ++sl) _Pragma("unroll") for (int cb = 0; cb < 2; ++cb) acc[S0][sl][cb] = f32x4{0.0f, 0.0f, 0.0f, 0.0f}; }
#define MH_HW_ZOUT(S2, Q)                                                                             \
    {                                                                                                 \
        char* const zb_ = zs_ + ((Q) & 1) * HWG_ZB + zwr;                                             \
        _Pragma("unroll") for (int cb = 0; cb < 2; ++cb) {                                            \
            *reinterpret_cast<f32x4*>(zb_ + cb * 2048) = acc[S2][0][cb] + acc[S2][1][cb];             \
            *reinterpret_cast<f32x4*>(zb_ + cb * 2048 + 1024) = acc[S2][1][cb];                       \
        }                                                                                             \
    }
#define MH_HW_FINISH(Q, ON)                                                                           \
    {                                                                                                 \
        const bool on_ = (ON);                                                                        \
        const char* const zb_ = zs_ + ((Q) & 1) * HWG_ZB + zrd;                                       \
        f32x2 z0_[3], z1_[3];                                                                         \
        _Pragma("unroll") for (int i = 0; i < 3; ++i) {                                               \
            z0_[i] = *reinterpret_cast<const f32x2*>(zb_ + i * 4096) + *reinterpret_cast<const f32x2*>(zb_ + i * 4096 + 16384 + 1024);        \
            z1_[i] = *reinterpret_cast<const f32x2*>(zb_ + i * 4096 + 1024) - *reinterpret_cast<const f32x2*>(zb_ + i * 4096 + 16384);        \
        }                                                                                             \
        const f32x2 fs_ = {fs2, fs2};                                                                 \
        const f32x2 y0_ = __builtin_elementwise_fma(z0_[2], fs_, __builtin_elementwise_fma(z0_[1], fs_, z0_[0])) * inv_a; \
        const f32x2 y1_ = __builtin_elementwise_fma(z1_[2], fs_, __builtin_elementwise_fma(z1_[1], fs_, z1_[0])) * inv_a; \
        f32x4 o_ = {__builtin_fmaf(y0_[0], inv_b, bco), __builtin_fmaf(y1_[0], inv_b, bco), __builtin_fmaf(y0_[1], inv_b, bco), __builtin_fmaf(y1_[1], inv_b, bco)}; \
        if (ACC) o_ += pv;       \
        __builtin_amdgcn_raw_buffer_store_b128(__builtin_bit_cast(u32x4, o_), orsrc, on_ ? ooff + (unsigned)(Q) * (unsigned)(HW * 4) : HWG_DROP, 0, 0); \
        if (STATS) {         \
            pivot = (on_ && !have_c) ? o_[0] : pivot;                                                 \
            have_c = have_c || on_;                                                                   \
            const f32x4 d_ = o_ - pivot, dw_ = d_ * (on_ ? 1.0f : 0.0f);                              \
            s1 += dw_;                                                                                \
            s2 = __builtin_elementwise_fma(dw_, d_, s2);                                              \
        }                                                                                             \
        if (POOL && !(HWX_OFF & 32)) {          \
            const f32x2 mx_ = {fmaxf(o_[0], o_[1]), fmaxf(o_[2], o_[3])}, mn_ = {fminf(o_[0], o_[1]), fminf(o_[2], o_[3])}; \
            const f32x2 own_ = fa ? mn_ : mx_, snd_ = fa ? mx_ : mn_;                                 \
            const f32x2 rcv_ = {hw_xchg32(snd_[0], fa), hw_xchg32(snd_[1], fa)};                      \
            const f32x2 y_ = {__builtin_amdgcn_fmed3f(own_[0], rcv_[0], pk_), __builtin_amdgcn_fmed3f(own_[1], rcv_[1], pk_)};       \
            const f32x2 f_ = {__builtin_amdgcn_fmed3f(y_[0], hm[0], pk_), __builtin_amdgcn_fmed3f(y_[1], hm[1], pk_)}; \
            const unsigned po_ = (on_ && ((Q) & 1) && !(HWX_OFF & 64)) ? poff + (unsigned)((Q) >> 1) * (unsigned)(PHW * 4) : HWG_DROP; \
            __builtin_amdgcn_raw_buffer_store_b64(__builtin_bit_cast(u32x2, f_), prs, po_, 0, 0);     \
            hm = on_ ? y_ : hm;                                                                       \
        }                                                                                             \
    }
#ifdef HWX_PROF
#define MH_HW_T(K) { const long long t_ = __builtin_readcyclecounter(); tacc[K] += t_ - tlast; tlast = t_; }
    long long tacc[8] = {0, 0, 0, 0, 0, 0, 0, 0}, tlast = __builtin_readcyclecounter();
#else
#define MH_HW_T(K)
#endif
#ifndef HWX_OFF
#define HWX_OFF 0
#endif
#ifndef HWX_DEAL
#define HWX_DEAL 2
#endif
#define MH_HW_DEAL                                                                                    \
    if constexpr (ACC || POOL) {                                                                      \
        _Pragma("unroll") for (int g_ = 0; g_ < 36; ++g_) {                                           \
            __builtin_amdgcn_sched_group_barrier(0x008, 1, 0);                                        \
            __builtin_amdgcn_sched_group_barrier(0x100, 1, 0);                                        \
            __builtin_amdgcn_sched_group_barrier(0x006, HWX_DEAL, 0);                                 \
            __builtin_amdgcn_sched_group_barrier(0x230, 1, 0);                                        \
        }                                                                                             \
    }
#define MH_HW_ITER(P, R)                                                                              \
    {                                                                                                 \
        constexpr int S0 = (3 - (R)) % 3, S1 = (S0 + 1) % 3, S2 = (S0 + 2) % 3;       \
        constexpr int db0 = (R) * HWG_DB, db2 = (((R) + 2) % 3) * HWG_DB;             \
        const int p_ = (P);                                                                           \
        const bool valid_ = p_ >= p_first && p_ <= p_last;                                            \
        const int qf_ = p_ - 2;                                                                       \
        if (ACC) { const bool nx_ = qf_ >= zs && qf_ < ze; pv = __builtin_bit_cast(f32x4, __builtin_amdgcn_raw_buffer_load_b128(orsrc, nx_ ? ooff + (unsigned)qf_ * hw4 : HWG_DROP, 0, 0)); } \
        if (valid_) { if (!(HWX_OFF & 1)) MH_HW_XFORM(db0) }                                          \
        MH_HW_T(0)                                                                                    \
        __syncthreads();                                                                              \
        MH_HW_T(1)                                                                                    \
        if (valid_) {                                                                                 \
            __builtin_amdgcn_sched_barrier(0);                                                        \
            if (!(HWX_OFF & 2)) { MH_HW_CONV(db2) MH_HW_LDX MH_HW_ADV }                               \
            if (!(HWX_OFF & 4)) MH_HW_FINISH(qf_, qf_ >= zs && qf_ < ze)                              \
            if (!(HWX_OFF & 8)) MH_HW_MMS(S0, S1, S2)                                                 \
            MH_HW_DEAL                                                                                \
            __builtin_amdgcn_sched_barrier(0);                                                        \
        } else {                                                                                      \
            MH_HW_SKIP(S0)                                                                            \
            if (!(HWX_OFF & 4)) MH_HW_FINISH(qf_, qf_ >= zs && qf_ < ze)                              \
        }                                                                                             \
        if (!(HWX_OFF & 16)) if (p_ - 1 >= zs && p_ - 1 < ze) MH_HW_ZOUT(S2, p_ - 1)                  \
        MH_HW_T(2)                                                                                    \
        __syncthreads();                                                                              \
        MH_HW_T(3)                                                                                    \
    }

    {
        const int k0 = p_first - (zs - 1);
        MH_HW_LDX MH_HW_ADV
        __syncthreads();
        MH_HW_CONV((k0 % 3) * HWG_DB)
        MH_HW_LDX MH_HW_ADV
        MH_HW_CONV(((k0 + 1) % 3) * HWG_DB)
        MH_HW_LDX MH_HW_ADV
        __syncthreads();
    }
    if (jp) __syncthreads();
    for (int p = zs - 1; p <= ze + 1; p += 3) {
        MH_HW_ITER(p, 0)
        MH_HW_ITER(p + 1, 1)
        MH_HW_ITER(p + 2, 2)
    }
    if (!jp) __syncthreads();
#ifdef HWX_PROF
    if (blockIdx.x == 0 && lane == 0) { _Pragma("unroll") for (int k = 0; k < 8; ++k) reinterpret_cast<long long*>(pmax)[wave * 8 + k] = tacc[k]; }
#endif
#undef MH_HW_T
#undef MH_HW_DEAL
#undef MH_HW_ITER
#undef MH_HW_FINISH
#undef MH_HW_ZOUT
#undef MH_HW_SKIP
#undef MH_HW_MMS
#undef MH_HW_MM
#undef MH_HW_XFORM
#undef MH_HW_U
#undef MH_HW_ADV
#undef MH_HW_CONV
#undef MH_HW_LDX

    if (STATS) {
        Stat run;
        {
            const float a1 = (s1[0] + s1[1]) + (s1[2] + s1[3]), a2 = (s2[0] + s2[1]) + (s2[2] + s2[3]);
            run.n = 4.0f * (float)(ze - zs);
            const float dm = a1 / run.n;
            run.mean = pivot + dm;
            run.m2 = fmaxf(a2 - a1 * dm, 0.0f);
        }
#pragma unroll
        for (int o = 16; o <= 32; o <<= 1) {
            Stat ot;
            ot.n = __shfl_xor(run.n, o); ot.mean = __shfl_xor(run.mean, o); ot.m2 = __shfl_xor(run.m2, o);
            run = (lane & o) == 0 ? stat_merge(run, ot) : stat_merge(ot, run);
        }
        __syncthreads();
        float* red = reinterpret_cast<float*>(smem);
        if (lane < 16) { red[(wave * 16 + lane) * 3] = run.n; red[(wave * 16 + lane) * 3 + 1] = run.mean; red[(wave * 16 + lane) * 3 + 2] = run.m2; }
        __syncthreads();
        if (tid < HWG_CN) {
            const int cb = tid >> 4, c16 = tid & 15;
            Stat st;
            st.n = 0.0f; st.mean = 0.0f; st.m2 = 0.0f;
#pragma unroll
            for (int w = 0; w < 4; ++w) {
                Stat ot;
                ot.n = red[((4 * cb + w) * 16 + c16) * 3]; ot.mean = red[((4 * cb + w) * 16 + c16) * 3 + 1]; ot.m2 = red[((4 * cb + w) * 16 + c16) * 3 + 2];
                st = stat_merge(st, ot);
            }
            float* rec = stats + (((long long)n * Cout + cg * HWG_CN + tid) * nblk + b) * 3;
            rec[0] = st.n; rec[1] = st.mean; rec[2] = st.m2;
        }
    }
}

__global__ void conv3d_k3_h2w_scale_fix_kernel(float* __restrict__ tail) {
    if (threadIdx.x == 0 && blockIdx.x == 0) { tail[0] *= 4.0f; tail[1] *= 0.25f; }
}
__global__ void __launch_bounds__(256)
conv3d_k3_h2w_pack_kernel(const float* __restrict__ w, int Cin, int Cout, _Float16* __restrict__ packed, const float* __restrict__ tail) {
    const int idx = blockIdx.x * 256 + threadIdx.x;
    if (idx >= Cin * Cout) return;
    const int ci = idx % Cin, co = idx / Cin;
    const float s = tail[1];
    const double G[4][3] = {{1.0, 0.0, 0.0}, {0.5, 0.5, 0.5}, {0.5, -0.5, 0.5}, {0.0, 0.0, 1.0}};
    const int cg = co / HWG_CN, cb = (co % HWG_CN) / 16, nn = co % 16;
    const int kg = ci < 16 ? ci / 4 : (ci - 16) / 4, e = ci < 16 ? ci % 4 : 4 + (ci - 16) % 4;
    const int ln = kg * 16 + nn;
    for (int t = 0; t < 3; ++t) {
        double g[3][3], tm[4][3];
        for (int ky = 0; ky < 3; ++ky)
            for (int kx = 0; kx < 3; ++kx) g[ky][kx] = (double)w[((long long)co * Cin + ci) * 27 + t * 9 + ky * 3 + kx];
        for (int i = 0; i < 4; ++i)
            for (int kx = 0; kx < 3; ++kx) tm[i][kx] = G[i][0] * g[0][kx] + G[i][1] * g[1][kx] + G[i][2] * g[2][kx];
        for (int i = 0; i < 4; ++i)
            for (int j = 0; j < 4; ++j) {
                const double u = tm[i][0] * G[j][0] + tm[i][1] * G[j][1] + tm[i][2] * G[j][2];
                _Float16 pc[2];
                h2_split((float)(u * (double)s), pc[0], pc[1]);
                const int jpq = j >> 1, slot = (j == 0 || j == 3) ? 0 : 1;
                for (int p = 0; p < 2; ++p) {
                    const long long r = (((long long)(cg * 8 + jpq * 4 + i) * HWG_OPS) + ((slot * 3 + t) * 2 + cb) * 2 + p) * 64 + ln;
                    packed[r * 8 + e] = pc[p];
                }
            }
    }
}

}
```

### monai_amd/networks/nets/basic_unet.py

```python

from __future__ import annotations

import threading
from collections.abc import Sequence
from typing import Optional

import torch
import torch.nn as nn

from ... import _lib, _prof, config, ops

__all__ = ["BasicUNet", "BasicUnet", "Basicunet", "basicunet"]


_BUILD = threading.local()


def _nd(three, two):
    return two if getattr(_BUILD, "dims", 3) == 2 else three


def _w5(w: torch.Tensor) -> torch.Tensor:
    return w if w.dim() == 5 else w.unsqueeze(2)

# ... 104 lines not shown
    if kind == "batch":
        return kind, {k: v for k, v in args.items() if k in ("eps", "momentum", "affine", "track_running_stats")}
    if kind == "group":
        if "num_groups" not in args:
            raise TypeError("GroupNorm.__init__() missing 1 required positional argument: 'num_groups'")
        return kind, {k: v for k, v in args.items() if k in ("num_groups", "eps", "affine")}
    raise NotImplementedError(f"monai_amd.BasicUNet: norm {norm!r} is not on the HIP path yet (instance / batch / group are)")


class BasicUNet(nn.Module):
    def __init__(
        self,
        spatial_dims: int = 3,
        in_channels: int = 1,
        out_channels: int = 2,
        features: Sequence[int] = (32, 32, 64, 128, 256, 32),
        act: str | tuple = ("LeakyReLU", {"negative_slope": 0.1, "inplace": True}),
        norm: str | tuple = ("instance", {"affine": True}),
        bias: bool = True,
        dropout: float | tuple = 0.0,
        upsample: str = "deconv",
    ):
        super().__init__()
        if spatial_dims not in (2, 3):
            raise NotImplementedError("monai_amd.BasicUNet: spatial_dims 2 and 3 are on the HIP path")
        if upsample not in ("deconv", "nontrainable", "pixelshuffle"):
            raise NotImplementedError("monai_amd.BasicUNet: upsample='deconv', 'nontrainable' and 'pixelshuffle' are on the HIP path")
        fea = tuple(features)
        if len(fea) != 6:
            raise ValueError(f"Sequence must have length 6, got length {len(fea)}.")
        print(f"BasicUNet features: {fea}.")
        slope = _parse_act(act)
        kw = dict(bias=bias, norm=_parse_norm(norm), slope=slope)
        self.features, self.in_channels, self.out_channels = fea, in_channels, out_channels
        self.spatial_dims, self.upsample = spatial_dims, upsample
        _BUILD.dims = spatial_dims
        try:
            self._build(in_channels, out_channels, fea, kw)
        finally:
            _BUILD.dims = 3
        self._plans: dict = {}
        self._packed: dict = {}
        self.fused_stats = True

    def _build(self, in_channels, out_channels, fea, kw):
        self.conv_0 = _TwoConv(in_channels, fea[0], **kw)
        self.down_1 = _Down(fea[0], fea[1], **kw)
        self.down_2 = _Down(fea[1], fea[2], **kw)
        self.down_3 = _Down(fea[2], fea[3], **kw)
        self.down_4 = _Down(fea[3], fea[4], **kw)
        up = self.upsample
        self.upcat_4 = _UpCat(fea[4], fea[3], fea[3], upsample=up, **kw)
        self.upcat_3 = _UpCat(fea[3], fea[2], fea[2], upsample=up, **kw)
        self.upcat_2 = _UpCat(fea[2], fea[1], fea[1], upsample=up, **kw)
        self.upcat_1 = _UpCat(fea[1], fea[0], fea[5], halves=False, upsample=up, **kw)
        self.final_conv = _nd(nn.Conv3d, nn.Conv2d)(fea[5], out_channels, kernel_size=1)

    def _packed_weight(self, name: str, conv: nn.Conv3d, cfg: int) -> torch.Tensor:
        w = conv.weight
        key = (w.data_ptr(), w._version, str(w.device))
        hit = self._packed.get((name, cfg))
        if hit is None or hit[0] != key:
            if w.dim() == 4:
                w3 = torch.zeros(w.shape[:2] + (3, 3, 3), dtype=w.dtype, device=w.device)
                w3[:, :, 1] = w
                w = w3
            hit = (key, ops.conv3d_k3_pack(cfg, w))
            self._packed[(name, cfg)] = hit
        return hit[1]

    def forward(self, x: torch.Tensor) -> torch.Tensor:
        if torch.is_grad_enabled() and x.requires_grad:
            raise NotImplementedError("monai_amd.BasicUNet: gradients w.r.t. the input are not on the (inference-only) HIP path")
        _lib.require_device(x)
        if self.spatial_dims == 2:
            if x.dim() != 4 or x.shape[1] != self.in_channels:
                raise RuntimeError(f"monai_amd.BasicUNet: expected input (B,{self.in_channels},H,W), got {tuple(x.shape)}")
            out = torch.empty((x.shape[0], self.out_channels) + tuple(x.shape[2:]), dtype=torch.float32, device=x.device)
            return self.forward_into(x, out)
        if x.dim() != 5 or x.shape[1] != self.in_channels:
            raise RuntimeError(f"monai_amd.BasicUNet: expected input (B,{self.in_channels},D,H,W), got {tuple(x.shape)}")
        out = torch.empty((x.shape[0], self.out_channels) + tuple(x.shape[2:]), dtype=torch.float32, device=x.device)
        return self.forward_into(x, out)

    @torch.no_grad()
    def forward_into(self, x: torch.Tensor, out: torch.Tensor) -> torch.Tensor:
        _lib.require_device(x, out[0].flat if isinstance(out, tuple) else out)
        if self.spatial_dims == 2 and x.dim() == 4 and not isinstance(out, tuple) and out.dim() == 4:
            self.forward_into(x.unsqueeze(2), out.unsqueeze(2))
            return out
        if self.training:
            raise NotImplementedError("monai_amd.BasicUNet: training mode (autograd) is not on the HIP path -- the engine is inference-only; with MONAI installed the call falls through to the reference module, which shares these parameters")
        x = x.contiguous()
        n, _, d, h, w = x.shape
        if self.spatial_dims == 2 and d != 1:
            raise RuntimeError(f"monai_amd.BasicUNet: a 2-D network takes one plane, got {tuple(x.shape)}")
        if min((h, w) if self.spatial_dims == 2 else (d, h, w)) < 16:
            raise RuntimeError(f"monai_amd.BasicUNet: window {d}x{h}x{w} is too small for four 2x poolings")
        key = (n, d, h, w, str(x.device))
        plan = self._plans.get(key)
        if plan is None:
            if len(self._plans) >= 4:
                self._plans.clear()
            plan = self._plans[key] = _Plan(self, n, (d, h, w), x.device)
        plan.run(self, x, out)
        return out


    @torch.no_grad()
    def forward_into_windows(self, x: torch.Tensor, mosaic, w0: int) -> None:
        self.forward_into(x, (mosaic, int(w0)))


BasicUnet = Basicunet = basicunet = BasicUNet


class _Plan:

    def __init__(self, net: "BasicUNet", n: int, dims, device):
        f = net.features
        self.n, self.dims = n, tuple(dims)
        self.planar = net.spatial_dims == 2
        self.sp = [tuple(v if (self.planar and a == 0) else v >> l for a, v in enumerate(dims)) for l in range(5)]
        up = [f[1], f[2] // 2, f[3] // 2, f[4] // 2]
        dec_out = [f[5], f[1], f[2], f[3]]
        e = lambda c, l: torch.empty((n, c) + self.sp[l], dtype=torch.float32, device=device)
        nz = lambda c: torch.zeros((n, c, 4), dtype=torch.float32, device=device)
        self.cat = [e(f[l] + up[l], l) for l in range(4)]
        self.cat_nrm = [nz(f[l] + up[l]) for l in range(4)]
        for l in range(4):
            self.cat_nrm[l][:, f[l]:, 0] = 1.0
            self.cat_nrm[l][:, f[l]:, 2] = 1.0
        self.tmp = [e(max(f[l], dec_out[l]) if l < 4 else f[4], l) for l in range(5)]
        self.tmp_nrm = [nz(max(f[l], dec_out[l]) if l < 4 else f[4]) for l in range(5)]
        self.pool = [None] + [e(f[l - 1], l) for l in range(1, 5)]
        self.pool_min = [None] * 5
        self.pool_nrm = [None] + [nz(f[l - 1]) for l in range(1, 5)]
        self.odd = [any(v & 1 for a, v in enumerate(self.sp[l]) if not (self.planar and a == 0)) for l in range(4)]
        self.up_scratch = [torch.empty((n, up[l]) + tuple(v if (self.planar and a == 0) else 2 * v for a, v in enumerate(self.sp[l + 1])),
                                       dtype=torch.float32, device=device)
                           if self.odd[l] else None for l in range(4)]
        self.up_scratch_nrm = [nz(up[l]) if self.odd[l] else None for l in range(4)]
        self.x4, self.x4_nrm = e(f[4], 4), nz(f[4])
        self.u = [e(dec_out[l], l) for l in range(4)]
        self.u_nrm = [nz(dec_out[l]) for l in range(4)]
        self.up, self.dec_out = up, dec_out
        self.batchnorm = isinstance(net.conv_0.conv_0.adn.N, (nn.BatchNorm3d, nn.BatchNorm2d))
        self.interp = net.upsample == "nontrainable"
        self.shuffle = net.upsample == "pixelshuffle"
        self.sub = [e((4 if self.planar else 8) * up[l], l + 1) if self.shuffle else None for l in range(4)]
        self.low = [e(up[l], l + 1) if self.interp else None for l in range(4)]
        self.stats: Optional[torch.Tensor] = None
        self.device = device

    def _stats_buf(self, floats: int) -> torch.Tensor:
        if self.stats is None or self.stats.numel() < floats:
            self.stats = torch.empty(floats, dtype=torch.float32, device=self.device)
        return self.stats

    def _bn_record(self, net, name: str, bn, slope: float, out_nrm) -> None:
        if bn.running_mean is None or bn.running_var is None:
            raise NotImplementedError("monai_amd.BasicUNet: BatchNorm without running statistics is not on the (inference) HIP path")
        parts = [bn.running_mean, bn.running_var] + ([bn.weight, bn.bias] if bn.affine else [])
        key = tuple((t.data_ptr(), t._version) for t in parts) + (slope, str(bn.running_mean.device))
        hit = net._packed.get(("bn", name))
        if hit is None or hit[0] != key:
            invstd = 1.0 / torch.sqrt(bn.running_var.float() + bn.eps)
            alpha = invstd * bn.weight.float() if bn.affine else invstd
            beta = (bn.bias.float() if bn.affine else 0.0) - bn.running_mean.float() * alpha
            hit = (key, torch.stack([alpha, beta, torch.full_like(alpha, slope), torch.zeros_like(alpha)], dim=1).contiguous())
            net._packed[("bn", name)] = hit
        out_nrm.copy_(hit[1][None].expand(out_nrm.shape[0], -1, -1))

    def _conv(self, net, name: str, block: _Convolution, x, x_nrm, out, out_nrm, bounded: bool = True, pool_level: int = 0) -> bool:
        n, cout, d, h, w = out.shape
        cin = x.shape[1]
        cfg = ops.conv3d_k3_select(cin, cout, d, h, w, bounded=x_nrm is not None and bounded and not self.batchnorm)
        packed = net._packed_weight(name, block.conv, cfg)
        norm = block.adn.N
        if pool_level and block.adn.negative_slope >= 0.0 and self._poolable(net, cfg, cin, cout, d, h, w, pool_level, x_nrm):
            if self.pool_min[pool_level] is None:
                self.pool_min[pool_level] = torch.empty_like(self.pool[pool_level])
            tiles = ops.conv3d_k3_stat_tiles(cfg, d, h, w)
            stats = self._stats_buf(n * cout * tiles * 3)
            with _prof.span(f"conv3d_k3/cfg{cfg}", 2.0 * 27 * cin * cout * d * h * w * n):
                ops.conv3d_k3_pool(cfg, x, x_nrm, packed, block.conv.bias, out, stats, self.pool[pool_level], self.pool_min[pool_level])
            if isinstance(norm, nn.GroupNorm):
                ops.groupnorm_finalize(stats, tiles, n, cout, norm.num_groups, norm.weight, norm.bias, norm.eps, block.adn.negative_slope, out_nrm)
            else:
                ops.instnorm_finalize(stats, tiles, n, cout, norm.weight, norm.bias, norm.eps, block.adn.negative_slope, out_nrm)
            ops.pool_select(self.pool[pool_level], self.pool_min[pool_level], out_nrm)
            return True
        if self.batchnorm:
            with _prof.span(f"conv3d_k3/cfg{cfg}", 2.0 * 27 * cin * cout * d * h * w * n):
                ops.conv3d_k3(cfg, x, x_nrm, packed, block.conv.bias, out, None)
            self._bn_record(net, name, norm, block.adn.negative_slope, out_nrm)
            return False
        tiles = ops.conv3d_k3_stat_tiles(cfg, d, h, w) if net.fused_stats else 0
        flops = 2.0 * 27 * cin * cout * d * h * w * n
        if tiles:
            stats = self._stats_buf(n * cout * tiles * 3)
            with _prof.span(f"conv3d_k3/cfg{cfg}", flops):
                ops.conv3d_k3(cfg, x, x_nrm, packed, block.conv.bias, out, stats)
        else:
            with _prof.span(f"conv3d_k3/cfg{cfg}", flops):
                ops.conv3d_k3(cfg, x, x_nrm, packed, block.conv.bias, out, None)
            tiles = ops.instnorm_stat_tiles(d, h, w)
            stats = self._stats_buf(n * cout * tiles * 3)
            ops.instnorm_stats(out, stats)
        if isinstance(norm, nn.GroupNorm):
            ops.groupnorm_finalize(stats, tiles, n, cout, norm.num_groups, norm.weight, norm.bias, norm.eps, block.adn.negative_slope, out_nrm)
        else:
            ops.instnorm_finalize(stats, tiles, n, cout, norm.weight, norm.bias, norm.eps, block.adn.negative_slope, out_nrm)
        return False

    def _halves_cfg(self, net, l: int, cout: int, bounded: bool) -> int:
        f = net.features
        if not config.conv_halves() or self.batchnorm or not net.fused_stats or not bounded or 2 * f[l] != int(self.cat[l].shape[1]):
            return -1
        _, _, d, h, w = self.cat[l].shape
        cfg = ops.conv3d_k3_select(f[l], cout, d, h, w, bounded=True)
        if cfg != ops.conv3d_k3_h2w_config() or ops.conv3d_k3_select(2 * f[l], cout, d, h, w, bounded=True) == cfg:
            return -1
        return cfg

    def _conv_halves(self, net, name: str, block: _Convolution, l: int, cfg: int, out, out_nrm) -> None:
        f = net.features
        fl = f[l]
        conv = block.conv
        n, cout, d, h, w = out.shape
        key = (conv.weight.data_ptr(), conv.weight._version, str(conv.weight.device))
        hit = net._packed.get(("halves", name, cfg))
        if hit is None or hit[0] != key:
            hit = (key, ops.conv3d_k3_pack(cfg, conv.weight[:, :fl].contiguous()), ops.conv3d_k3_pack(cfg, conv.weight[:, fl:].contiguous()))
            net._packed[("halves", name, cfg)] = hit
        flops = 2.0 * 27 * fl * cout * d * h * w * n
        with _prof.span(f"conv3d_k3/cfg{cfg}", flops):
            ops.conv3d_k3(cfg, self.cat[l][:, :fl], self.cat_nrm[l][:, :fl], hit[1], None, out, None)
        tiles = ops.conv3d_k3_stat_tiles(cfg, d, h, w)
        stats = self._stats_buf(n * cout * tiles * 3)
        with _prof.span(f"conv3d_k3/cfg{cfg}", flops):
            ops.conv3d_k3(cfg, self.cat[l][:, fl:], self.cat_nrm[l][:, fl:], hit[2], conv.bias, out, stats, accumulate=True)
        norm = block.adn.N
        if isinstance(norm, nn.GroupNorm):
            ops.groupnorm_finalize(stats, tiles, n, cout, norm.num_groups, norm.weight, norm.bias, norm.eps, block.adn.negative_slope, out_nrm)
        else:
            ops.instnorm_finalize(stats, tiles, n, cout, norm.weight, norm.bias, norm.eps, block.adn.negative_slope, out_nrm)

    def _poolable(self, net, cfg: int, cin: int, cout: int, d: int, h: int, w: int, level: int, x_nrm) -> bool:
        if self.planar or self.batchnorm or not net.fused_stats or x_nrm is None or not config.pool_fused():
            return False
        if tuple(self.sp[level]) != (d // 2, h // 2, w // 2) or tuple(self.pool[level].shape[1:]) != (cout, d // 2, h // 2, w // 2):
            return False
        return ops.conv3d_k3_pool_accepts(cfg, cin, cout, d, h, w)

    def _interpolate(self, up: _UpSample, src, src_nrm, low, dst) -> None:
        if hasattr(up, "preconv"):
            pc = up.preconv
            ops.conv1x1(src, src_nrm, pc.weight.view(pc.weight.shape[0], -1), pc.bias, low)
        else:
            ops.add_act(src, src_nrm, None, None, 1.0, low)
        n, c, d, h, w = low.shape
        osz = (d if self.planar else 2 * d, 2 * h, 2 * w)
        a = [1.0 if (self.planar or d == 1) else (d - 1) / (osz[0] - 1), (h - 1) / (osz[1] - 1), (w - 1) / (osz[2] - 1)]
        m = [a[0], 0, 0, 0, 0, a[1], 0, 0, 0, 0, a[2], 0]
        hi = ops.affine_resample(low.reshape(n * c, d, h, w), m, osz, "bilinear", "border", False, False)
        dst.copy_(hi.reshape((n, c) + osz))

    def _subpixel(self, net, name: str, conv: nn.Conv3d, src, src_nrm, sub, dst, dst_nrm) -> None:
        n, cin, d, h, w = src.shape
        cout = sub.shape[1]
        cfg = ops.conv3d_k3_select(cin, cout, d, h, w, bounded=src_nrm is not None and not self.batchnorm)
        with _prof.span(f"conv3d_k3/cfg{cfg}", 2.0 * 27 * cin * cout * d * h * w * n):
            ops.conv3d_k3(cfg, src, src_nrm, net._packed_weight(name, conv, cfg), conv.bias, sub, None)
        ops.pixelshuffle(sub, dst, 1 if self.planar else 2, True, dst_nrm)

    def _fusable(self, net, l: int, src: torch.Tensor, cout: int) -> bool:
        if self.interp or self.shuffle or self.planar or self.odd[l] or self.batchnorm or not net.fused_stats or not config.upcat_fused():
            return False
        if config.conv_algo() not in (config.CONV_ALGOS["auto"], config.CONV_ALGOS["h2"]):
            return False
        return ops.upconv_k4s2_accepts(int(src.shape[1]), int(cout), *self.sp[l + 1])

    def _upcat_fused(self, net, l: int, upc: "_UpCat", src, src_nrm, out, out_nrm) -> None:
        f = net.features
        block, name = upc.convs.conv_0, f"upcat_{l + 1}.convs.conv_0"
        conv, dec = block.conv, upc.upsample.deconv
        n, cout, d, h, w = out.shape
        skip, skip_nrm = self.cat[l][:, : f[l]], self.cat_nrm[l][:, : f[l]]
        parts = [conv.weight, dec.weight] + ([dec.bias] if dec.bias is not None else [])
        key = tuple((p_.data_ptr(), p_._version) for p_ in parts) + (str(conv.weight.device),)
        cfg = ops.conv3d_k3_select(f[l], cout, d, h, w, bounded=True)
        hit = net._packed.get(("upcat", name, cfg))
        if hit is None or hit[0] != key:
            w4, table = ops.upconv_k4s2_weights(dec.weight, dec.bias, conv.weight[:, f[l]:])
            hit = (key, ops.conv3d_k3_pack(cfg, conv.weight[:, : f[l]].contiguous()), ops.upconv_k4s2_pack(w4), table)
            net._packed[("upcat", name, cfg)] = hit
        _, packed_skip, packed_up, table = hit
        up_flops = 2.0 * 8 * int(src.shape[1]) * cout * d * h * w * n
        if cfg in (ops.conv3d_k3_h2_config(), ops.conv3d_k3_h2w_config()) and config.upcat_order() == "term_first":
            with _prof.span("upconv_k4s2", up_flops):
                ops.upconv_k4s2(src, src_nrm, packed_up, table, out, accumulate=False)
            tiles = ops.conv3d_k3_stat_tiles(cfg, d, h, w)
            stats = self._stats_buf(n * cout * tiles * 3)
            with _prof.span(f"conv3d_k3/cfg{cfg}", 2.0 * 27 * f[l] * cout * d * h * w * n):
                ops.conv3d_k3(cfg, skip, skip_nrm, packed_skip, conv.bias, out, stats, accumulate=True)
        else:
            with _prof.span(f"conv3d_k3/cfg{cfg}", 2.0 * 27 * f[l] * cout * d * h * w * n):
                ops.conv3d_k3(cfg, skip, skip_nrm, packed_skip, conv.bias, out, None)
            tiles = ops.upconv_k4s2_stat_tiles(*self.sp[l + 1])
            stats = self._stats_buf(n * cout * tiles * 3)
            with _prof.span("upconv_k4s2", up_flops):
                ops.upconv_k4s2(src, src_nrm, packed_up, table, out, accumulate=True, stats=stats)
        norm = block.adn.N
        if isinstance(norm, nn.GroupNorm):
            ops.groupnorm_finalize(stats, tiles, n, cout, norm.num_groups, norm.weight, norm.bias, norm.eps, block.adn.negative_slope, out_nrm)
        else:
            ops.instnorm_finalize(stats, tiles, n, cout, norm.weight, norm.bias, norm.eps, block.adn.negative_slope, out_nrm)

    def run(self, net: "BasicUNet", x: torch.Tensor, logits: torch.Tensor) -> None:
        f = net.features
        downs = [None, net.down_1, net.down_2, net.down_3, net.down_4]
        ups = [net.upcat_1, net.upcat_2, net.upcat_3, net.upcat_4]

        t, tn = self.tmp[0][:, : f[0]], self.tmp_nrm[0][:, : f[0]]
        self._conv(net, "conv_0.conv_0", net.conv_0.conv_0, x, None, t, tn)
        pooled = self._conv(net, "conv_0.conv_1", net.conv_0.conv_1, t, tn, self.cat[0][:, : f[0]], self.cat_nrm[0][:, : f[0]], pool_level=1)
        for l in range(1, 5):
            skip, skip_nrm = self.cat[l - 1][:, : f[l - 1]], self.cat_nrm[l - 1][:, : f[l - 1]]
            if pooled:
                p_in, p_nrm = self.pool[l], skip_nrm
            else:
                ops.maxpool2(skip, skip_nrm, self.pool[l], self.pool_nrm[l])
                p_in, p_nrm = self.pool[l], self.pool_nrm[l]
            t, tn = self.tmp[l][:, : f[l]], self.tmp_nrm[l][:, : f[l]]
            self._conv(net, f"down_{l}.convs.conv_0", downs[l].convs.conv_0, p_in, p_nrm, t, tn)
            if l < 4:
                o, on = self.cat[l][:, : f[l]], self.cat_nrm[l][:, : f[l]]
            else:
                o, on = self.x4, self.x4_nrm
            pooled = self._conv(net, f"down_{l}.convs.conv_1", downs[l].convs.conv_1, t, tn, o, on, pool_level=l + 1 if l < 4 else 0)

        src, src_nrm = self.x4, self.x4_nrm
        for l in range(3, -1, -1):
            upc = ups[l]
            co = self.dec_out[l]
            t, tn = self.tmp[l][:, :co], self.tmp_nrm[l][:, :co]
            if self._fusable(net, l, src, co):
                self._upcat_fused(net, l, upc, src, src_nrm, t, tn)
            else:
                dst = self.up_scratch[l] if self.odd[l] else self.cat[l][:, f[l]:]
                dst_nrm = ops.nrm_identity(self.up_scratch_nrm[l] if self.odd[l] else self.cat_nrm[l][:, f[l]:])
                if self.interp:
                    self._interpolate(upc.upsample, src, src_nrm, self.low[l], dst)
                elif self.shuffle:
                    self._subpixel(net, f"upcat_{l + 1}.upsample.pixelshuffle.conv_block", upc.upsample.pixelshuffle.conv_block, src, src_nrm, self.sub[l], dst, dst_nrm)
                elif self.planar:
                    ops.deconv_ks(src, src_nrm, _w5(upc.upsample.deconv.weight).contiguous(), upc.upsample.deconv.bias, dst, (1, 2, 2), dst_nrm)
                else:
                    ops.deconv_k2s2(src, src_nrm, upc.upsample.deconv.weight, upc.upsample.deconv.bias, dst, dst_nrm, bounded=src_nrm is not None and not self.batchnorm)
                if self.odd[l]:
                    ops.pad_replicate(self.up_scratch[l], self.cat[l][:, f[l]:], self.up_scratch_nrm[l], self.cat_nrm[l][:, f[l]:])
                hcfg = self._halves_cfg(net, l, co, bounded=not self.interp)
                if hcfg >= 0:
                    self._conv_halves(net, f"upcat_{l + 1}.convs.conv_0", upc.convs.conv_0, l, hcfg, t, tn)
                else:
                    self._conv(net, f"upcat_{l + 1}.convs.conv_0", upc.convs.conv_0, self.cat[l], self.cat_nrm[l], t, tn, bounded=not self.interp)
            self._conv(net, f"upcat_{l + 1}.convs.conv_1", upc.convs.conv_1, t, tn, self.u[l], self.u_nrm[l])
            src, src_nrm = self.u[l], self.u_nrm[l]

        fc = net.final_conv
        if isinstance(logits, tuple):
            ops.conv1x1_windows(src, src_nrm, fc.weight.view(fc.weight.shape[0], -1), fc.bias, logits[0], logits[1])
        else:
            ops.conv1x1(src, src_nrm, fc.weight.view(fc.weight.shape[0], -1), fc.bias, logits)
```

### monai_amd/ops.py

```python

from __future__ import annotations

import ctypes as C
from typing import Optional, Sequence

import torch

from . import _lib

Grid = Sequence[Sequence[int]]


def _s(t):
    return _lib.stream_ptr(t)


def window_extract(vol: torch.Tensor, grid: Grid, w0: int, nwin: int, roi: Sequence[int], out: torch.Tensor) -> torch.Tensor:
    _lib.require_device(vol, out)
    if vol.dim() != 4 or not vol.is_contiguous() or not out.is_contiguous():
        raise RuntimeError("monai_amd.window_extract: vol must be a contiguous [C,D,H,W] tensor")
    c, d, h, w = vol.shape
    sz, sy, sx = grid
    _lib.lib().call(
        "mh_window_extract_f32", _lib.ptr(vol), c, d, h, w, _lib.int_array(sz), len(sz), _lib.int_array(sy), len(sy),
# ... 152 lines not shown
            n = len(starts)
            if n > 1 and any(starts[i] != i * starts[1] for i in range(n - 1)):
                return False
            if n > 2 and cls.residue_log2(n, starts[1], r) is None:
                return False
        return True

    def __init__(self, grid, roi, k: int, device, dtype=torch.float32, allocate: bool = True):
        self.grid, self.roi, self.k = [list(g) for g in grid], tuple(int(v) for v in roi), int(k)
        self.n = [len(g) for g in self.grid]
        self.log2m = [self.residue_log2(n, g[1] if n > 1 else 1, r) for n, g, r in zip(self.n, self.grid, self.roi)]
        self.cnt = []
        for n, lg in zip(self.n, self.log2m):
            c = (C.c_int32 * self.CLASSES)()
            _lib.lib().call("mh_sw_mosaic_class_counts", int(n), int(lg), c)
            self.cnt.append([int(v) for v in c])
        self.base = [0] * self.CLASSES ** 3
        total = 0
        for cz in range(self.CLASSES):
            for cy in range(self.CLASSES):
                for cx in range(self.CLASSES):
                    size = self.k * self.cnt[0][cz] * self.roi[0] * self.cnt[1][cy] * self.roi[1] * self.cnt[2][cx] * self.roi[2]
                    self.base[(cz * self.CLASSES + cy) * self.CLASSES + cx] = total
                    if size:
                        total = (total + size + 3) // 4 * 4
                        if size * 4 >= (1 << 20):
                            total = (total + 63) // 64 * 64 + 17 * 64
        self.total, self._device, self._dtype = max(total, 4), device, dtype
        self.flat = None
        if allocate:
            self.allocate()

    def allocate(self):
        self.flat = torch.empty(self.total, dtype=self._dtype, device=self._device)
        return self

    def place(self, w: int):
        nz, ny, nx = self.n
        idx = (w // (ny * nx), (w // nx) % ny, w % nx)
        cls, j = [], []
        for a in range(3):
            last = idx[a] == self.n[a] - 1
            m = 1 << self.log2m[a]
            cls.append(m if last else idx[a] & (m - 1))
            j.append(0 if last else idx[a] >> self.log2m[a])
        dc, hc, wc = (self.cnt[a][cls[a]] * self.roi[a] for a in range(3))
        off = self.base[(cls[0] * self.CLASSES + cls[1]) * self.CLASSES + cls[2]] + ((j[0] * self.roi[0]) * hc + j[1] * self.roi[1]) * wc + j[2] * self.roi[2]
        return off, dc * hc * wc, hc * wc, wc

    def window_view(self, w: int) -> torch.Tensor:
        off, sc, sd, sh = self.place(w)
        return self.flat.as_strided((self.k,) + self.roi, (sc, sd, sh, 1), off)

    def places(self, w0: int, n: int):
        flat = [int(v) for w in range(w0, w0 + n) for v in self.place(w)]
        return (C.c_int64 * len(flat))(*flat)


def sw_blend_mosaic(mosaic: LogitsMosaic, imp: torch.Tensor, out: torch.Tensor) -> torch.Tensor:
    _lib.require_device(mosaic.flat, imp, out)
    if not (imp.is_contiguous() and out.is_contiguous()):
        raise RuntimeError("monai_amd.sw_blend_mosaic: contiguous tensors required")
    factored = imp.dim() == 1
    if factored and imp.numel() != sum(mosaic.roi) + 1:
        raise RuntimeError("monai_amd.sw_blend_mosaic: factored importance map must hold rd + rh + rw + 1 floats")
    k, d, h, w = out.shape
    sz, sy, sx = mosaic.grid
    _lib.lib().call("mh_sw_blend_mosaic_f32", _lib.ptr(mosaic.flat), (C.c_int64 * len(mosaic.base))(*mosaic.base), *[int(v) for v in mosaic.log2m], _lib.ptr(imp),
                    int(factored), _lib.ptr(out), k, d, h, w, *mosaic.roi, _lib.int_array(sz), len(sz), _lib.int_array(sy), len(sy), _lib.int_array(sx), len(sx), _s(out))
    return out


def conv1x1_windows(x, x_nrm, weight, bias, mosaic: LogitsMosaic, w0: int):
    _lib.require_device(x, x_nrm, weight, bias, mosaic.flat)
    xi = _lib.tensor5(x, x_nrm)
    _lib.lib().call("mh_conv1x1_windows_f32", C.byref(xi), _lib.ptr(weight), _lib.ptr(bias), _lib.ptr(mosaic.flat), int(weight.shape[0]),
                    mosaic.places(int(w0), int(x.shape[0])), _s(x))


def conv3d_k3_select(cin: int, cout: int, d: int, h: int, w: int, bounded: bool = False, algo: Optional[int] = None) -> int:
    from . import config

    cfg = _lib.lib().query("mh_conv3d_k3_select", config.conv_algo() if algo is None else int(algo), int(bool(bounded)), cin, cout, d, h, w)
    if not config.small_volume_h2() and cfg == _lib.lib().query("mh_conv3d_k3_h2v_config"):
        cfg = _lib.lib().query("mh_conv3d_k3_select", config.CONV_ALGOS["fp32"], int(bool(bounded)), cin, cout, d, h, w)
    return cfg


def conv3d_k3_num_configs() -> int:
    return _lib.lib().query("mh_conv3d_k3_num_configs")


def conv3d_k3_h2_config() -> int:
    return _lib.lib().query("mh_conv3d_k3_h2_config")


def conv3d_k3_h2c_config() -> int:
    return _lib.lib().query("mh_conv3d_k3_h2c_config")


def conv3d_k3_c1_config() -> int:
    return _lib.lib().query("mh_conv3d_k3_c1_config")


def conv3d_k3_h2v_config() -> int:
    return _lib.lib().query("mh_conv3d_k3_h2v_config")


def conv3d_k3_h2w_config() -> int:
    return _lib.lib().query("mh_conv3d_k3_h2w_config")


def conv3d_k3_h2w_fits(d: int, h: int, w: int) -> bool:
    return bool(_lib.lib().query("mh_conv3d_k3_h2w_fits", int(d), int(h), int(w)))


def conv3d_k3_accepts(cfg: int, cin: int, cout: int) -> bool:
    return bool(_lib.lib().query("mh_conv3d_k3_accepts", int(cfg), int(cin), int(cout)))


def conv3d_k3_pack(cfg: int, weight: torch.Tensor) -> torch.Tensor:
    _lib.require_device(weight)
    cout, cin = weight.shape[:2]
    wc = weight.detach().contiguous()
    packed = torch.empty(_lib.lib().query("mh_conv3d_k3_packed_floats", cfg, cin, cout), dtype=torch.float32, device=weight.device)
    _lib.lib().call("mh_conv3d_k3_pack_f32", cfg, _lib.ptr(wc), cin, cout, _lib.ptr(packed), _s(weight))
    return packed


def conv3d_k3_stat_tiles(cfg: int, d: int, h: int, w: int) -> int:
    return _lib.lib().query("mh_conv3d_k3_stat_tiles", cfg, d, h, w)


def conv3d_k3(cfg, x, x_nrm, packed_w, bias, out, stats: Optional[torch.Tensor] = None, accumulate: bool = False):
    _lib.require_device(x, x_nrm, packed_w, bias, out, stats)
    xi, xo = _lib.tensor5(x, x_nrm), _lib.tensor5(out)
    _lib.lib().call("mh_conv3d_k3_accumulate_f32" if accumulate else "mh_conv3d_k3_f32", int(cfg), C.byref(xi), _lib.ptr(packed_w), _lib.ptr(bias), C.byref(xo),
                    _lib.ptr(stats), _s(x))
    return out


def conv3d_k3_pool_accepts(cfg: int, cin: int, cout: int, d: int, h: int, w: int) -> bool:
    return bool(_lib.lib().query("mh_conv3d_k3_pool_accepts", int(cfg), int(cin), int(cout), int(d), int(h), int(w)))


def conv3d_k3_pool(cfg, x, x_nrm, packed_w, bias, out, stats, pool_max: torch.Tensor, pool_min: torch.Tensor):
    _lib.require_device(x, x_nrm, packed_w, bias, out, stats, pool_max, pool_min)
    if pool_max.shape != pool_min.shape or pool_max.stride() != pool_min.stride() or not pool_max[0].is_contiguous():
        raise RuntimeError("monai_amd.conv3d_k3_pool: pool_max / pool_min must be two equally laid out [N, C, D/2, H/2, W/2] tensors, dense per sample")
    xi, xo = _lib.tensor5(x, x_nrm), _lib.tensor5(out)
    _lib.lib().call("mh_conv3d_k3_pool_f32", int(cfg), C.byref(xi), _lib.ptr(packed_w), _lib.ptr(bias), C.byref(xo), _lib.ptr(stats), _lib.ptr(pool_max), _lib.ptr(pool_min),
                    int(pool_max.stride(0)), _s(x))
    return out


def pool_select(pool_max: torch.Tensor, pool_min: torch.Tensor, nrm: torch.Tensor) -> torch.Tensor:
    _lib.require_device(pool_max, pool_min, nrm)
    n, c = int(pool_max.shape[0]), int(pool_max.shape[1])
    vol = int(pool_max.shape[2] * pool_max.shape[3] * pool_max.shape[4])
    if nrm.dim() != 3 or nrm.shape[2] != 4 or nrm.stride(2) != 1 or nrm.stride(1) != 4:
        raise RuntimeError("monai_amd.pool_select: nrm must be an [N, C, 4] record view")
    _lib.lib().call("mh_pool_select_f32", _lib.ptr(pool_max), _lib.ptr(pool_min), _lib.ptr(nrm), int(nrm.stride(0)), n, c, int(pool_max.stride(0)), vol, _s(pool_max))
    return pool_max


def instnorm_stat_tiles(d: int, h: int, w: int) -> int:
    return _lib.lib().query("mh_instnorm_stat_tiles", d, h, w)


def instnorm_stats(x: torch.Tensor, stats: torch.Tensor):
    _lib.require_device(x, stats)
    xi = _lib.tensor5(x)
    _lib.lib().call("mh_instnorm_stats_f32", C.byref(xi), _lib.ptr(stats), _s(x))
    return stats


def instnorm_finalize(stats, tiles: int, n: int, c: int, gamma, beta, eps: float, slope: float, nrm: torch.Tensor):
    _lib.require_device(stats, gamma, beta, nrm)
    if nrm.dim() != 3 or nrm.shape[2] != 4 or nrm.stride(2) != 1 or nrm.stride(1) != 4:
        raise RuntimeError("monai_amd.instnorm_finalize: nrm must be a [N,C,4] slice")
    ns = nrm.stride(0) if n > 1 else max(nrm.stride(0), 4 * c)
    _lib.lib().call(
        "mh_instnorm_finalize_f32", _lib.ptr(stats), int(tiles), int(n), int(c), _lib.ptr(gamma), _lib.ptr(beta), float(eps),
        float(slope), _lib.ptr(nrm), int(ns), _s(stats),
    )
    return nrm


def nrm_identity(nrm: torch.Tensor) -> torch.Tensor:
    _lib.require_device(nrm)
    if nrm.dim() != 3 or nrm.shape[2] != 4 or nrm.stride(2) != 1 or nrm.stride(1) != 4:
        raise RuntimeError("monai_amd.nrm_identity: nrm must be a [N,C,4] slice")
    n, c = nrm.shape[:2]
    _lib.lib().call("mh_nrm_identity_f32", _lib.ptr(nrm), int(n), int(c), int(nrm.stride(0) if n > 1 else max(nrm.stride(0), 4 * c)), _s(nrm))
    return nrm


def maxpool2(x, x_nrm, out, out_nrm=None):
    _lib.require_device(x, x_nrm, out, out_nrm)
    xi, xo = _lib.tensor5(x, x_nrm), _lib.tensor5(out, out_nrm)
    _lib.lib().call("mh_maxpool2_f32", C.byref(xi), C.byref(xo), _s(x))
    return out


_DECONV_H2_PACKED: dict = {}


def deconv_k2s2_h2_packed(weight: torch.Tensor) -> torch.Tensor:
    import weakref

    hit = _DECONV_H2_PACKED.get(id(weight))
    if hit is None or hit[0]() is not weight or hit[1] != weight._version or hit[2] != str(weight.device) or hit[3] != weight.data_ptr():
        if len(_DECONV_H2_PACKED) > 256:
            for k in [k for k, v in _DECONV_H2_PACKED.items() if v[0]() is None]:
                del _DECONV_H2_PACKED[k]
        cin, cout = int(weight.shape[0]), int(weight.shape[1])
        packed = torch.zeros(_lib.lib().query("mh_deconv_k2s2_h2_packed_floats", cin, cout), dtype=torch.float32, device=weight.device)
        _lib.lib().call("mh_deconv_k2s2_h2_pack_f32", _lib.ptr(weight.detach().contiguous()), cin, cout, _lib.ptr(packed), _s(weight))
        hit = (weakref.ref(weight), weight._version, str(weight.device), weight.data_ptr(), packed)
        _DECONV_H2_PACKED[id(weight)] = hit
    return hit[4]


def deconv_k2s2(x, x_nrm, weight, bias, out, out_nrm=None, bounded: bool = False):
    _lib.require_device(x, x_nrm, weight, bias, out, out_nrm)
    xi, xo = _lib.tensor5(x, x_nrm), _lib.tensor5(out, out_nrm)
    if bounded and x_nrm is not None and tuple(weight.shape[2:]) == (2, 2, 2):
        from . import config

        cin, cout = int(weight.shape[0]), int(weight.shape[1])
        if config.deconv_h2() and _lib.lib().query("mh_deconv_k2s2_h2_accepts", cin, cout, int(x.shape[2]), int(x.shape[3]), int(x.shape[4])):
            _lib.lib().call("mh_deconv_k2s2_h2_f32", C.byref(xi), _lib.ptr(deconv_k2s2_h2_packed(weight)), _lib.ptr(bias), C.byref(xo), _s(x))
            return out
    _lib.lib().call("mh_deconv_k2s2_f32", C.byref(xi), _lib.ptr(weight), _lib.ptr(bias), C.byref(xo), _s(x))
    return out


def upconv_k4s2_accepts(cin: int, cout: int, dl: int, hl: int, wl: int) -> bool:
    return bool(_lib.lib().query("mh_upconv_k4s2_accepts", int(cin), int(cout), int(dl), int(hl), int(wl)))


def upconv_k4s2_weights(deconv_w: torch.Tensor, deconv_b: Optional[torch.Tensor], conv_w_up: torch.Tensor):
    wd, wc = deconv_w.detach().float(), conv_w_up.detach().float()
    cin, cout = wd.shape[0], wc.shape[0]
    pairs = {-1: ((0, 2),), 0: ((0, 1), (1, 2)), 1: ((0, 0), (1, 1)), 2: ((1, 0),)}
    w4 = torch.zeros((cin, cout, 4, 4, 4), dtype=torch.float32, device=wd.device)
    for uz, pz_ in pairs.items():
        for uy, py_ in pairs.items():
            for ux, px_ in pairs.items():
                acc = None
                for dz, kz in pz_:
                    for dy, ky in py_:
                        for dx, kx in px_:
                            t = wd[:, :, dz, dy, dx] @ wc[:, :, kz, ky, kx].t()
                            acc = t if acc is None else acc + t
                w4[:, :, uz + 1, uy + 1, ux + 1] = acc
    inside = ((1, 2), (0, 1, 2), (0, 1))
    table = torch.zeros((27, cout), dtype=torch.float32, device=wd.device)
    if deconv_b is not None:
        bd = deconv_b.detach().float()
        for cz in range(3):
            for cy in range(3):
                for cx in range(3):
                    wsum = wc[:, :, list(inside[cz])][:, :, :, list(inside[cy])][:, :, :, :, list(inside[cx])].sum(dim=(2, 3, 4))
                    table[(cz * 3 + cy) * 3 + cx] = wsum @ bd
    return w4.contiguous(), table.contiguous()


def upconv_k4s2_pack(w4: torch.Tensor) -> torch.Tensor:
    _lib.require_device(w4)
    cin, cout = int(w4.shape[0]), int(w4.shape[1])
    packed = torch.zeros(_lib.lib().query("mh_upconv_k4s2_packed_floats", cin, cout), dtype=torch.float32, device=w4.device)
    _lib.lib().call("mh_upconv_k4s2_pack_f32", _lib.ptr(w4.contiguous()), cin, cout, _lib.ptr(packed), _s(w4))
    return packed


def upconv_k4s2_stat_tiles(dl: int, hl: int, wl: int) -> int:
    return _lib.lib().query("mh_upconv_k4s2_stat_tiles", int(dl), int(hl), int(wl))


def upconv_k4s2(low, low_nrm, packed, bias_table, out, accumulate: bool = False, stats=None):
    _lib.require_device(low, low_nrm, packed, bias_table, out, stats)
    xi, xo = _lib.tensor5(low, low_nrm), _lib.tensor5(out)
    _lib.lib().call("mh_upconv_k4s2_f32", C.byref(xi), _lib.ptr(packed), _lib.ptr(bias_table), C.byref(xo), int(bool(accumulate)), _lib.ptr(stats), _s(out))
    return out


def conv1x1_stat_tiles(d: int, h: int, w: int) -> int:
    return _lib.lib().query("mh_conv1x1_stat_tiles", d, h, w)


def conv1x1(x, x_nrm, weight, bias, out, stats=None):
    _lib.require_device(x, x_nrm, weight, bias, out, stats)
    xi, xo = _lib.tensor5(x, x_nrm), _lib.tensor5(out)
    if stats is None:
        _lib.lib().call("mh_conv1x1_f32", C.byref(xi), _lib.ptr(weight), _lib.ptr(bias), C.byref(xo), _s(x))
    else:
        _lib.lib().call("mh_conv1x1_stats_f32", C.byref(xi), _lib.ptr(weight), _lib.ptr(bias), C.byref(xo), _lib.ptr(stats), _s(x))
    return out


def conv1x1_h2_accepts(cin: int, cout: int, d: int, h: int, w: int) -> bool:
    return bool(_lib.lib().query("mh_conv1x1_h2_accepts", int(cin), int(cout), int(d), int(h), int(w)))


def conv1x1_h2_wanted(cin: int, cout: int, d: int, h: int, w: int) -> bool:
# ... 411 lines not shown
```

Before: 206.0 million voxels/s.

## Add blocked-16 channel activation layout to the Winograd split conv path

```diff
diff --git a/include/monai_amd.h b/include/monai_amd.h
--- a/include/monai_amd.h
+++ b/include/monai_amd.h
@@ -77,6 +77,9 @@
                           int64_t pool_n_stride, void* stream);
 int mh_pool_select_f32(float* pool_max, const float* pool_min, const float* nrm, int64_t nrm_n_stride, int N, int C, int64_t n_stride, int64_t vol, void* stream);
 int mh_conv3d_k3_accumulate_f32(int cfg, const mh_tensor5* in, const float* packed_w, const float* bias, const mh_tensor5* out, float* stats, void* stream);
+int mh_conv3d_k3_blk_accepts(int cfg, int in_block, int out_block);
+int mh_conv3d_k3_blk_f32(int cfg, const mh_tensor5* in, int in_block, const float* packed_w, const float* bias, const mh_tensor5* out, int out_block, float* stats,
+                         int accumulate, float* pool_max, float* pool_min, int64_t pool_n_stride, void* stream);
 
 int mh_instnorm_stat_tiles(int D, int H, int W);
 int mh_instnorm_stats_f32(const mh_tensor5* x, float* stats, void* stream);
diff --git a/monai_amd/_lib.py b/monai_amd/_lib.py
--- a/monai_amd/_lib.py
+++ b/monai_amd/_lib.py
@@ -65,6 +65,8 @@
     "mh_conv3d_k3_stat_tiles": (_I, [_I, _I, _I, _I]),
     "mh_conv3d_k3_f32": (_I, [_I, _T, _P, _P, _T, _P, _P]),
     "mh_conv3d_k3_accumulate_f32": (_I, [_I, _T, _P, _P, _T, _P, _P]),
+    "mh_conv3d_k3_blk_accepts": (_I, [_I, _I, _I]),
+    "mh_conv3d_k3_blk_f32": (_I, [_I, _T, _I, _P, _P, _T, _I, _P, _I, _P, _P, _L, _P]),
     "mh_conv3d_k3_pool_accepts": (_I, [_I, _I, _I, _I, _I, _I]),
     "mh_conv3d_k3_pool_f32": (_I, [_I, _T, _P, _P, _T, _P, _P, _P, _L, _P]),
     "mh_pool_select_f32": (_I, [_P, _P, _P, _L, _I, _I, _L, _L, _P]),
diff --git a/monai_amd/config.py b/monai_amd/config.py
--- a/monai_amd/config.py
+++ b/monai_amd/config.py
@@ -76,6 +76,16 @@
     return str(v).lower() not in ("0", "false", "off", "no")
 
 
+ACT_LAYOUT = None
+
+
+def act_layout() -> str:
+    v = str(ACT_LAYOUT if ACT_LAYOUT is not None else os.environ.get("MONAI_AMD_ACT_LAYOUT", "auto")).lower()
+    if v not in ("auto", "ncdhw"):
+        raise ValueError(f"monai_amd: unknown activation layout {v!r} (auto or ncdhw)")
+    return v
+
+
 STRIDED_H2 = None
 
 
diff --git a/monai_amd/csrc/capi.hip b/monai_amd/csrc/capi.hip
--- a/monai_amd/csrc/capi.hip
+++ b/monai_amd/csrc/capi.hip
@@ -609,7 +609,7 @@
 
 struct PoolOut { float* mx; float* mn; long long n_stride; };
 static int conv3d_k3_launch(int cfg, const mh_tensor5* in_, const float* packed_w, const float* bias, const mh_tensor5* out_, float* stats, void* stream, bool accumulate,
-                            const PoolOut* pool = nullptr);
+                            const PoolOut* pool = nullptr, bool in_blk = false, bool out_blk = false);
 int mh_conv3d_k3_pool_accepts(int cfg, int Cin, int Cout, int D, int H, int W);
 int mh_conv3d_k3_pool_f32(int cfg, const mh_tensor5* in_, const float* packed_w, const float* bias, const mh_tensor5* out_, float* stats, float* pool_max, float* pool_min,
                           int64_t pool_n_stride, void* stream) {
@@ -637,8 +637,36 @@
         return fail(MH_ERR_UNSUPPORTED, "conv3d_k3_accumulate: the accumulating form exists for the split-precision configuration with input records and statistics");
     return conv3d_k3_launch(cfg, in_, packed_w, bias, out_, stats, stream, true);
 }
+int mh_conv3d_k3_blk_accepts(int cfg, int in_block, int out_block) {
+    if ((in_block != 0 && in_block != 16) || (out_block != 0 && out_block != 16)) return 0;
+    return (in_block == 0 && out_block == 0) || cfg == MH_CFG_H2W;
+}
+int mh_conv3d_k3_blk_f32(int cfg, const mh_tensor5* in_, int in_block, const float* packed_w, const float* bias, const mh_tensor5* out_, int out_block, float* stats,
+                         int accumulate, float* pool_max, float* pool_min, int64_t pool_n_stride, void* stream) {
+    if ((in_block != 0 && in_block != 16) || (out_block != 0 && out_block != 16))
+        return fail(MH_ERR_ARG, "conv3d_k3_blk: the channel block width is 0 (NCDHW) or 16 (got %d, %d)", in_block, out_block);
+    if (!in_ || !out_) return fail(MH_ERR_ARG, "conv3d_k3_blk: bad tensor");
+    if (!mh_conv3d_k3_blk_accepts(cfg, in_block, out_block))
+        return fail(MH_ERR_UNSUPPORTED, "conv3d_k3_blk: configuration %d has no blocked-16 form (the Winograd split configuration has)", cfg);
+    if ((in_block && in_->C % 16) || (out_block && out_->C % 16)) return fail(MH_ERR_ARG, "conv3d_k3_blk: a blocked tensor has a multiple of 16 channels (got %d, %d)", in_->C, out_->C);
+    if ((in_block && (!aligned(in_->data, 64) || in_->n_stride % 16)) || (out_block && (!aligned(out_->data, 64) || out_->n_stride % 16)))
+        return fail(MH_ERR_ARG, "conv3d_k3_blk: a blocked view starts on a block boundary (64-byte aligned data, batch stride a multiple of 16 floats)");
+    if ((pool_max != nullptr) != (pool_min != nullptr) || (accumulate && pool_max)) return fail(MH_ERR_ARG, "conv3d_k3_blk: both pooled tensors or none; not with accumulate");
+    if (pool_max) {
+        if (!stats || !in_->nrm) return fail(MH_ERR_ARG, "conv3d_k3_blk: the pooling form needs input records and statistics");
+        if (!mh_conv3d_k3_pool_accepts(cfg, in_->C, out_->C, out_->D, out_->H, out_->W)) return fail(MH_ERR_UNSUPPORTED, "conv3d_k3_blk: no pooling epilogue for this layer");
+        if (!aligned(pool_max, 8) || !aligned(pool_min, 8) || pool_n_stride % 2 || (long long)out_->C * (out_->D / 2) * (out_->H / 2) * (out_->W / 2) > pool_n_stride)
+            return fail(MH_ERR_ARG, "conv3d_k3_blk: pooled tensors must be 8-byte aligned [N][>= C][D/2][H/2][W/2]");
+        const PoolOut po{pool_max, pool_min, (long long)pool_n_stride};
+        return conv3d_k3_launch(cfg, in_, packed_w, bias, out_, stats, stream, false, &po, in_block != 0, out_block != 0);
+    }
+    if (accumulate && ((cfg != MH_CFG_H2 && cfg != MH_CFG_H2C && cfg != MH_CFG_H2W) || !stats || !in_->nrm))
+        return fail(MH_ERR_UNSUPPORTED, "conv3d_k3_blk: the accumulating form exists for the split-precision configuration with input records and statistics");
+    return conv3d_k3_launch(cfg, in_, packed_w, bias, out_, stats, stream, accumulate != 0, nullptr, in_block != 0, out_block != 0);
+}
 static int conv3d_k3_launch(int cfg, const mh_tensor5* in_, const float* packed_w, const float* bias, const mh_tensor5* out_,
-                            float* stats, void* stream, bool accumulate, const PoolOut* pool) {
+                            float* stats, void* stream, bool accumulate, const PoolOut* pool, bool in_blk, bool out_blk) {
+    if ((in_blk || out_blk) && cfg != MH_CFG_H2W) return fail(MH_ERR_UNSUPPORTED, "conv3d_k3: configuration %d has no blocked-16 form", cfg);
     if (!dense_ok(in_) || !dense_ok(out_) || !packed_w) return fail(MH_ERR_ARG, "conv3d_k3: bad tensor");
     const Tensor in = from_c(*in_), out = from_c(*out_);
     if (in.N != out.N || in.D != out.D || in.H != out.H || in.W != out.W) return fail(MH_ERR_ARG, "conv3d_k3: shape mismatch");
@@ -674,10 +702,18 @@
         const dim3 grid((unsigned)total);
         const uint4* wq = reinterpret_cast<const uint4*>(packed_w);
         const float* tail = packed_w + (mh_conv3d_k3_packed_floats(cfg, in.C, out.C) - H2_TAIL);
-        if (pool) hipLaunchKernelGGL((conv3d_k3_h2w_kernel<true, false, true>), grid, dim3(64 * HWG_WAVES), 0, s, in, wq, tail, bias, out, stats, bxn, byn, zc, nblk, pool->mx, pool->mn, pool->n_stride);
-        else if (accumulate) hipLaunchKernelGGL((conv3d_k3_h2w_kernel<true, true, false>), grid, dim3(64 * HWG_WAVES), 0, s, in, wq, tail, bias, out, stats, bxn, byn, zc, nblk, (float*)nullptr, (float*)nullptr, 0LL);
-        else if (stats) hipLaunchKernelGGL((conv3d_k3_h2w_kernel<true, false, false>), grid, dim3(64 * HWG_WAVES), 0, s, in, wq, tail, bias, out, stats, bxn, byn, zc, nblk, (float*)nullptr, (float*)nullptr, 0LL);
-        else hipLaunchKernelGGL((conv3d_k3_h2w_kernel<false, false, false>), grid, dim3(64 * HWG_WAVES), 0, s, in, wq, tail, bias, out, stats, bxn, byn, zc, nblk, (float*)nullptr, (float*)nullptr, 0LL);
+#define MH_HW_LAUNCH(BI_, BO_)                                                                                                                       \
+    {                                                                                                                                                \
+        if (pool) hipLaunchKernelGGL((conv3d_k3_h2w_kernel<true, false, true, BI_, BO_>), grid, dim3(64 * HWG_WAVES), 0, s, in, wq, tail, bias, out, stats, bxn, byn, zc, nblk, pool->mx, pool->mn, pool->n_stride); \
+        else if (accumulate) hipLaunchKernelGGL((conv3d_k3_h2w_kernel<true, true, false, BI_, BO_>), grid, dim3(64 * HWG_WAVES), 0, s, in, wq, tail, bias, out, stats, bxn, byn, zc, nblk, (float*)nullptr, (float*)nullptr, 0LL); \
+        else if (stats) hipLaunchKernelGGL((conv3d_k3_h2w_kernel<true, false, false, BI_, BO_>), grid, dim3(64 * HWG_WAVES), 0, s, in, wq, tail, bias, out, stats, bxn, byn, zc, nblk, (float*)nullptr, (float*)nullptr, 0LL); \
+        else hipLaunchKernelGGL((conv3d_k3_h2w_kernel<false, false, false, BI_, BO_>), grid, dim3(64 * HWG_WAVES), 0, s, in, wq, tail, bias, out, stats, bxn, byn, zc, nblk, (float*)nullptr, (float*)nullptr, 0LL); \
+    }
+        if (in_blk && out_blk) MH_HW_LAUNCH(true, true)
+        else if (in_blk) MH_HW_LAUNCH(true, false)
+        else if (out_blk) MH_HW_LAUNCH(false, true)
+        else MH_HW_LAUNCH(false, false)
+#undef MH_HW_LAUNCH
         return launched("conv3d_k3_h2w");
     }
     if (cfg == MH_CFG_H2V) {
diff --git a/monai_amd/csrc/kernels/common.h b/monai_amd/csrc/kernels/common.h
--- a/monai_amd/csrc/kernels/common.h
+++ b/monai_amd/csrc/kernels/common.h
@@ -122,6 +122,16 @@
     return r;
 }
 
+template <class Rsrc>
+__device__ __forceinline__ void buf_store_b32(const float v, const Rsrc r, const unsigned voffset, const unsigned soffset) {
+#ifdef MH_SIMT_EMULATOR
+    const unsigned long long off = (unsigned long long)voffset + soffset;
+    if (off + 4ull <= r.num_records) __builtin_memcpy(r.base + off, &v, 4);
+#else
+    __builtin_amdgcn_raw_buffer_store_b32(__builtin_bit_cast(unsigned, v), r, voffset, soffset, 0);
+#endif
+}
+
 __device__ __forceinline__ unsigned xcd_remap(unsigned b, unsigned nb) {
     const unsigned q = nb / 8u, r = nb % 8u, x = b % 8u, i = b / 8u;
     return (x < r ? x * (q + 1u) : r * (q + 1u) + (x - r) * q) + i;
diff --git a/monai_amd/csrc/kernels/conv3d_wino_h2.h b/monai_amd/csrc/kernels/conv3d_wino_h2.h
--- a/monai_amd/csrc/kernels/conv3d_wino_h2.h
+++ b/monai_amd/csrc/kernels/conv3d_wino_h2.h
@@ -64,7 +64,10 @@
 #define MH_HW_KEEP_BRANCH asm volatile("" ::: "memory")
 #endif
 
-template <bool STATS, bool ACC = false, bool POOL = false>
+#ifndef HWX_BLKI_LDS
+#define HWX_BLKI_LDS 2
+#endif
+template <bool STATS, bool ACC = false, bool POOL = false, bool BLKI = false, bool BLKO = false>
 __global__ void __launch_bounds__(512)
 conv3d_k3_h2w_kernel(Tensor in, const uint4* __restrict__ wp, const float* __restrict__ wtail, const float* __restrict__ bias, Tensor out,
                      float* __restrict__ stats, int bxn, int byn, int zchunk, unsigned nblk, float* __restrict__ pmax, float* __restrict__ pmin,
@@ -89,9 +92,22 @@
     const int zs = (int)(b / (bxn * byn)) * zchunk, ze = min(zs + zchunk, D);
     const int p_first = max(zs - 1, 0), p_last = min(ze, D - 1);
 
-    unsigned soff;
+    unsigned soff = 0u;
+    unsigned soffb[2] = {0u, 0u};
     int loff[2];
-    {
+    if constexpr (BLKI) {
+        const int q = lane & 3;
+#pragma unroll
+        for (int j = 0; j < 2; ++j) {
+            const int t = 64 * j + lane;
+            const int pos = 27 * (wave & 3) + (t >> 2);
+            const int ly = pos / HWG_RX, lx = pos - HWG_RX * ly;
+            const int gy = y0 + ly - 1, gx = x0 + lx - 1;
+            const bool ok = t < HWG_NP && gy >= 0 && gy < H && gx >= 0 && gx < W;
+            soffb[j] = ok ? 64u * (unsigned)(gy * W + gx) + 16u * (unsigned)q : 0u;
+            loff[j] = (ok ? pos : HWG_NP) * HWG_PB + (wave >> 2) * 64 + q * 16;
+        }
+    } else {
         const int pr = min(lane, 53);
         const int ly = pr / 9;
         int lx = 2 * (pr - 9 * ly);
@@ -126,20 +142,30 @@
         const float p_ = __uint_as_float((unsigned)(e_in + 127) << 23);
 #pragma unroll
         for (int i = 0; i < 4; ++i) {
-            const float4 a = *reinterpret_cast<const float4*>(in.nrm + (long long)n * in.nrm_n_stride + 4LL * (4 * wave + i));
+            const int c_ = BLKI ? (wave >> 2) * 16 + 4 * (lane & 3) + i : 4 * wave + i;
+            const float4 a = *reinterpret_cast<const float4*>(in.nrm + (long long)n * in.nrm_n_stride + 4LL * c_);
             nra[i] = a.x * p_; nrb[i] = a.y * p_; nrs[i] = a.z;
         }
     }
     f32x4 nrk;
 #pragma unroll
     for (int i = 0; i < 4; ++i) nrk[i] = nrs[i] <= 1.0f ? __builtin_inff() : -__builtin_inff();
-    const auto xrs = __builtin_amdgcn_make_buffer_rsrc(const_cast<float*>(in.data + (long long)n * in.n_stride + (long long)(4 * wave) * DHW), 0, 0x7fffffff, 0x00020000);
-    const unsigned hw4 = (unsigned)(HW * 4);
-    unsigned voff = soff + (unsigned)p_first * hw4;
+    const int rslot = ((wave >> 2) * 4 + (lane & 3)) * HWG_PB + 128;
+    if constexpr (BLKI) {
+        *reinterpret_cast<f32x4*>(ds + rslot) = nrk;
+        if (HWX_BLKI_LDS > 1) *reinterpret_cast<f32x4*>(ds + rslot + 8 * HWG_PB) = nrs;
+    }
+    const auto xrs = __builtin_amdgcn_make_buffer_rsrc(const_cast<float*>(in.data + (long long)n * in.n_stride + (long long)(BLKI ? (wave >> 2) * 16 : 4 * wave) * DHW), 0, 0x7fffffff, 0x00020000);
+    const unsigned hw4 = (unsigned)(HW * (BLKI ? 64 : 4));
+    unsigned voff = (BLKI ? 0u : soff) + (unsigned)p_first * hw4;
     const unsigned cso1 = (unsigned)(DHW * 4), cso2 = 2u * cso1, cso3 = 3u * cso1;
     f32x2 xin[4];
+    f32x4 xib[2];
 #define MH_HW_LDX                                                                                     \
-    {                                                                                                 \
+    if constexpr (BLKI) {                                                                             \
+        xib[0] = __builtin_bit_cast(f32x4, __builtin_amdgcn_raw_buffer_load_b128(xrs, soffb[0], voff, 0)); \
+        xib[1] = __builtin_bit_cast(f32x4, __builtin_amdgcn_raw_buffer_load_b128(xrs, soffb[1], voff, 0)); \
+    } else {                                                                                          \
         xin[0] = __builtin_bit_cast(f32x2, __builtin_amdgcn_raw_buffer_load_b64(xrs, voff, 0u, 0));   \
         xin[1] = __builtin_bit_cast(f32x2, __builtin_amdgcn_raw_buffer_load_b64(xrs, voff, cso1, 0)); \
         xin[2] = __builtin_bit_cast(f32x2, __builtin_amdgcn_raw_buffer_load_b64(xrs, voff, cso2, 0)); \
@@ -147,11 +173,15 @@
     }
 #define MH_HW_CONV(DBO)                                                                               \
     {                                                                                                 \
-        char* const db_ = ds + (DBO) + 16 * wave;                                                     \
+        char* const db_ = ds + (DBO) + (BLKI ? 0 : 16 * wave);                                        \
+        f32x4 k_ = nrk, s_ = nrs;                                                                     \
+        if constexpr (BLKI) { k_ = *reinterpret_cast<const f32x4*>(ds + rslot); if (HWX_BLKI_LDS > 1) s_ = *reinterpret_cast<const f32x4*>(ds + rslot + 8 * HWG_PB); } \
         _Pragma("unroll") for (int j = 0; j < 2; ++j) {                                               \
             f32x4 y_;                                                                                 \
-            const f32x4 t_ = __builtin_elementwise_fma(f32x4{xin[0][j], xin[1][j], xin[2][j], xin[3][j]}, nra, nrb), u_ = t_ * nrs; \
-            _Pragma("unroll") for (int i = 0; i < 4; ++i) y_[i] = __builtin_amdgcn_fmed3f(t_[i], u_[i], nrk[i]);       \
+            f32x4 x_;                                                                                 \
+            if constexpr (BLKI) x_ = xib[j]; else x_ = f32x4{xin[0][j], xin[1][j], xin[2][j], xin[3][j]}; \
+            const f32x4 t_ = __builtin_elementwise_fma(x_, nra, nrb), u_ = t_ * s_;                   \
+            _Pragma("unroll") for (int i = 0; i < 4; ++i) y_[i] = __builtin_amdgcn_fmed3f(t_[i], u_[i], k_[i]);       \
             *reinterpret_cast<f32x4*>(db_ + loff[j]) = y_;                                            \
         }                                                                                             \
     }
@@ -200,7 +230,9 @@
         inv_b = __uint_as_float((unsigned)(t2_ + 127) << 23);
     }
     const auto orsrc = __builtin_amdgcn_make_buffer_rsrc(out.data + (long long)n * out.n_stride + (long long)(cg * HWG_CN) * DHW, 0, (int)(HWG_CN * DHW * 4), 0x00020000);
-    const unsigned ooff = 4u * (unsigned)((long long)co_l * DHW + (long long)(y0 + 2 * fty + fa) * W + x0 + 2 * ftx);
+    const unsigned ooff = BLKO ? 4u * (unsigned)((((long long)fcb * DHW + (long long)(y0 + 2 * fty + fa) * W + x0 + 2 * ftx) << 4) + (il & 15))
+                               : 4u * (unsigned)((long long)co_l * DHW + (long long)(y0 + 2 * fty + fa) * W + x0 + 2 * ftx);
+    const unsigned hwo = (unsigned)(HW * (BLKO ? 64 : 4));
     float pivot = 0.0f;
     bool have_c = false;
     f32x4 s1 = {0.0f, 0.0f, 0.0f, 0.0f}, s2 = s1;
@@ -263,7 +295,9 @@
         const f32x2 y1_ = __builtin_elementwise_fma(z1_[2], fs_, __builtin_elementwise_fma(z1_[1], fs_, z1_[0])) * inv_a; \
         f32x4 o_ = {__builtin_fmaf(y0_[0], inv_b, bco), __builtin_fmaf(y1_[0], inv_b, bco), __builtin_fmaf(y0_[1], inv_b, bco), __builtin_fmaf(y1_[1], inv_b, bco)}; \
         if (ACC) o_ += pv;       \
-        __builtin_amdgcn_raw_buffer_store_b128(__builtin_bit_cast(u32x4, o_), orsrc, on_ ? ooff + (unsigned)(Q) * (unsigned)(HW * 4) : HWG_DROP, 0, 0); \
+        const unsigned so_ = on_ ? ooff + (unsigned)(Q) * hwo : HWG_DROP;                             \
+        if constexpr (BLKO) { _Pragma("unroll") for (int k = 0; k < 4; ++k) buf_store_b32(o_[k], orsrc, so_ + 64u * k, 0u); } \
+        else __builtin_amdgcn_raw_buffer_store_b128(__builtin_bit_cast(u32x4, o_), orsrc, so_, 0, 0); \
         if (STATS) {         \
             pivot = (on_ && !have_c) ? o_[0] : pivot;                                                 \
             have_c = have_c || on_;                                                                   \
@@ -310,7 +344,12 @@
         const int p_ = (P);                                                                           \
         const bool valid_ = p_ >= p_first && p_ <= p_last;                                            \
         const int qf_ = p_ - 2;                                                                       \
-        if (ACC) { const bool nx_ = qf_ >= zs && qf_ < ze; pv = __builtin_bit_cast(f32x4, __builtin_amdgcn_raw_buffer_load_b128(orsrc, nx_ ? ooff + (unsigned)qf_ * hw4 : HWG_DROP, 0, 0)); } \
+        if (ACC) {                                                                                    \
+            const bool nx_ = qf_ >= zs && qf_ < ze;                                                   \
+            const unsigned po_ = nx_ ? ooff + (unsigned)qf_ * hwo : HWG_DROP;                         \
+            if constexpr (BLKO) { _Pragma("unroll") for (int k = 0; k < 4; ++k) pv[k] = __builtin_bit_cast(float, __builtin_amdgcn_raw_buffer_load_b32(orsrc, po_ + 64u * k, 0u, 0)); } \
+            else pv = __builtin_bit_cast(f32x4, __builtin_amdgcn_raw_buffer_load_b128(orsrc, po_, 0, 0)); \
+        }                                                                                             \
         if (valid_) { if (!(HWX_OFF & 1)) MH_HW_XFORM(db0) }                                          \
         MH_HW_T(0)                                                                                    \
         __syncthreads();                                                                              \
diff --git a/monai_amd/networks/nets/basic_unet.py b/monai_amd/networks/nets/basic_unet.py
--- a/monai_amd/networks/nets/basic_unet.py
+++ b/monai_amd/networks/nets/basic_unet.py
@@ -280,6 +280,22 @@
         self.low = [e(up[l], l + 1) if self.interp else None for l in range(4)]
         self.stats: Optional[torch.Tensor] = None
         self.device = device
+        self.last_layouts = {"tmp0": 0, "skip0": 0, "u0": 0}
+
+    def _layouts(self, net) -> dict:
+        lay = {"tmp0": 0, "skip0": 0, "u0": 0}
+        if config.act_layout() != "auto" or self.planar or self.batchnorm or not net.fused_stats:
+            return lay
+        f = net.features
+        d, h, w = self.sp[0]
+        h2w = ops.conv3d_k3_h2w_config()
+        if f[0] % 16 or ops.conv3d_k3_select(f[0], f[0], d, h, w, bounded=True) != h2w or not ops.conv3d_k3_blk_accepts(h2w, 16, 16):
+            return lay
+        pooled = net.conv_0.conv_1.adn.negative_slope >= 0.0 and self._poolable(net, h2w, f[0], f[0], d, h, w, 1, True)
+        fused = self._fusable(net, 0, self.u[1], self.dec_out[0]) and ops.conv3d_k3_select(f[0], self.dec_out[0], d, h, w, bounded=True) == h2w
+        if pooled and fused:
+            lay["skip0"] = 16
+        return lay
 
     def _stats_buf(self, floats: int) -> torch.Tensor:
         if self.stats is None or self.stats.numel() < floats:
@@ -300,7 +316,7 @@
             net._packed[("bn", name)] = hit
         out_nrm.copy_(hit[1][None].expand(out_nrm.shape[0], -1, -1))
 
-    def _conv(self, net, name: str, block: _Convolution, x, x_nrm, out, out_nrm, bounded: bool = True, pool_level: int = 0) -> bool:
+    def _conv(self, net, name: str, block: _Convolution, x, x_nrm, out, out_nrm, bounded: bool = True, pool_level: int = 0, in_blk: int = 0, out_blk: int = 0) -> bool:
         n, cout, d, h, w = out.shape
         cin = x.shape[1]
         cfg = ops.conv3d_k3_select(cin, cout, d, h, w, bounded=x_nrm is not None and bounded and not self.batchnorm)
@@ -312,13 +328,18 @@
             tiles = ops.conv3d_k3_stat_tiles(cfg, d, h, w)
             stats = self._stats_buf(n * cout * tiles * 3)
             with _prof.span(f"conv3d_k3/cfg{cfg}", 2.0 * 27 * cin * cout * d * h * w * n):
-                ops.conv3d_k3_pool(cfg, x, x_nrm, packed, block.conv.bias, out, stats, self.pool[pool_level], self.pool_min[pool_level])
+                if in_blk or out_blk:
+                    ops.conv3d_k3_blk(cfg, x, x_nrm, packed, block.conv.bias, out, stats, in_blk, out_blk, pool_max=self.pool[pool_level], pool_min=self.pool_min[pool_level])
+                else:
+                    ops.conv3d_k3_pool(cfg, x, x_nrm, packed, block.conv.bias, out, stats, self.pool[pool_level], self.pool_min[pool_level])
             if isinstance(norm, nn.GroupNorm):
                 ops.groupnorm_finalize(stats, tiles, n, cout, norm.num_groups, norm.weight, norm.bias, norm.eps, block.adn.negative_slope, out_nrm)
             else:
                 ops.instnorm_finalize(stats, tiles, n, cout, norm.weight, norm.bias, norm.eps, block.adn.negative_slope, out_nrm)
             ops.pool_select(self.pool[pool_level], self.pool_min[pool_level], out_nrm)
             return True
+        if (in_blk or out_blk) and (self.batchnorm or not net.fused_stats or not ops.conv3d_k3_stat_tiles(cfg, d, h, w) or (pool_level and out_blk)):
+            raise RuntimeError(f"monai_amd.BasicUNet: {name} was planned on blocked-16 activations but takes a path that reads NCDHW")
         if self.batchnorm:
             with _prof.span(f"conv3d_k3/cfg{cfg}", 2.0 * 27 * cin * cout * d * h * w * n):
                 ops.conv3d_k3(cfg, x, x_nrm, packed, block.conv.bias, out, None)
@@ -329,7 +350,10 @@
         if tiles:
             stats = self._stats_buf(n * cout * tiles * 3)
             with _prof.span(f"conv3d_k3/cfg{cfg}", flops):
-                ops.conv3d_k3(cfg, x, x_nrm, packed, block.conv.bias, out, stats)
+                if in_blk or out_blk:
+                    ops.conv3d_k3_blk(cfg, x, x_nrm, packed, block.conv.bias, out, stats, in_blk, out_blk)
+                else:
+                    ops.conv3d_k3(cfg, x, x_nrm, packed, block.conv.bias, out, stats)
         else:
             with _prof.span(f"conv3d_k3/cfg{cfg}", flops):
                 ops.conv3d_k3(cfg, x, x_nrm, packed, block.conv.bias, out, None)
@@ -410,7 +434,7 @@
             return False
         return ops.upconv_k4s2_accepts(int(src.shape[1]), int(cout), *self.sp[l + 1])
 
-    def _upcat_fused(self, net, l: int, upc: "_UpCat", src, src_nrm, out, out_nrm) -> None:
+    def _upcat_fused(self, net, l: int, upc: "_UpCat", src, src_nrm, out, out_nrm, skip_blk: int = 0) -> None:
         f = net.features
         block, name = upc.convs.conv_0, f"upcat_{l + 1}.convs.conv_0"
         conv, dec = block.conv, upc.upsample.deconv
@@ -426,16 +450,24 @@
             net._packed[("upcat", name, cfg)] = hit
         _, packed_skip, packed_up, table = hit
         up_flops = 2.0 * 8 * int(src.shape[1]) * cout * d * h * w * n
+        if skip_blk and cfg != ops.conv3d_k3_h2w_config():
+            raise RuntimeError("monai_amd.BasicUNet: a blocked-16 skip tensor needs the Winograd split convolution on the UpCat's skip half")
         if cfg in (ops.conv3d_k3_h2_config(), ops.conv3d_k3_h2w_config()) and config.upcat_order() == "term_first":
             with _prof.span("upconv_k4s2", up_flops):
                 ops.upconv_k4s2(src, src_nrm, packed_up, table, out, accumulate=False)
             tiles = ops.conv3d_k3_stat_tiles(cfg, d, h, w)
             stats = self._stats_buf(n * cout * tiles * 3)
             with _prof.span(f"conv3d_k3/cfg{cfg}", 2.0 * 27 * f[l] * cout * d * h * w * n):
-                ops.conv3d_k3(cfg, skip, skip_nrm, packed_skip, conv.bias, out, stats, accumulate=True)
+                if skip_blk:
+                    ops.conv3d_k3_blk(cfg, skip, skip_nrm, packed_skip, conv.bias, out, stats, skip_blk, 0, accumulate=True)
+                else:
+                    ops.conv3d_k3(cfg, skip, skip_nrm, packed_skip, conv.bias, out, stats, accumulate=True)
         else:
             with _prof.span(f"conv3d_k3/cfg{cfg}", 2.0 * 27 * f[l] * cout * d * h * w * n):
-                ops.conv3d_k3(cfg, skip, skip_nrm, packed_skip, conv.bias, out, None)
+                if skip_blk:
+                    ops.conv3d_k3_blk(cfg, skip, skip_nrm, packed_skip, conv.bias, out, None, skip_blk, 0)
+                else:
+                    ops.conv3d_k3(cfg, skip, skip_nrm, packed_skip, conv.bias, out, None)
             tiles = ops.upconv_k4s2_stat_tiles(*self.sp[l + 1])
             stats = self._stats_buf(n * cout * tiles * 3)
             with _prof.span("upconv_k4s2", up_flops):
@@ -451,9 +483,12 @@
         downs = [None, net.down_1, net.down_2, net.down_3, net.down_4]
         ups = [net.upcat_1, net.upcat_2, net.upcat_3, net.upcat_4]
 
+        lay = self.last_layouts = self._layouts(net)
         t, tn = self.tmp[0][:, : f[0]], self.tmp_nrm[0][:, : f[0]]
-        self._conv(net, "conv_0.conv_0", net.conv_0.conv_0, x, None, t, tn)
-        pooled = self._conv(net, "conv_0.conv_1", net.conv_0.conv_1, t, tn, self.cat[0][:, : f[0]], self.cat_nrm[0][:, : f[0]], pool_level=1)
+        self._conv(net, "conv_0.conv_0", net.conv_0.conv_0, x, None, t, tn, out_blk=lay["tmp0"])
+        pooled = self._conv(net, "conv_0.conv_1", net.conv_0.conv_1, t, tn, self.cat[0][:, : f[0]], self.cat_nrm[0][:, : f[0]], pool_level=1, in_blk=lay["tmp0"], out_blk=lay["skip0"])
+        if lay["skip0"] and not pooled:
+            raise RuntimeError("monai_amd.BasicUNet: a blocked-16 skip tensor needs the pooling epilogue (the pooling pass reads NCDHW)")
         for l in range(1, 5):
             skip, skip_nrm = self.cat[l - 1][:, : f[l - 1]], self.cat_nrm[l - 1][:, : f[l - 1]]
             if pooled:
@@ -475,7 +510,7 @@
             co = self.dec_out[l]
             t, tn = self.tmp[l][:, :co], self.tmp_nrm[l][:, :co]
             if self._fusable(net, l, src, co):
-                self._upcat_fused(net, l, upc, src, src_nrm, t, tn)
+                self._upcat_fused(net, l, upc, src, src_nrm, t, tn, skip_blk=lay["skip0"] if l == 0 else 0)
             else:
                 dst = self.up_scratch[l] if self.odd[l] else self.cat[l][:, f[l]:]
                 dst_nrm = ops.nrm_identity(self.up_scratch_nrm[l] if self.odd[l] else self.cat_nrm[l][:, f[l]:])
diff --git a/monai_amd/ops.py b/monai_amd/ops.py
--- a/monai_amd/ops.py
+++ b/monai_amd/ops.py
@@ -328,6 +328,38 @@
     _lib.lib().call("mh_conv3d_k3_pool_f32", int(cfg), C.byref(xi), _lib.ptr(packed_w), _lib.ptr(bias), C.byref(xo), _lib.ptr(stats), _lib.ptr(pool_max), _lib.ptr(pool_min),
                     int(pool_max.stride(0)), _s(x))
     return out
+
+
+def conv3d_k3_blk_accepts(cfg: int, in_block: int = 0, out_block: int = 0) -> bool:
+    return bool(_lib.lib().query("mh_conv3d_k3_blk_accepts", int(cfg), int(in_block), int(out_block)))
+
+
+def conv3d_k3_blk(cfg, x, x_nrm, packed_w, bias, out, stats=None, in_block: int = 0, out_block: int = 0, accumulate: bool = False,
+                  pool_max: Optional[torch.Tensor] = None, pool_min: Optional[torch.Tensor] = None):
+    _lib.require_device(x, x_nrm, packed_w, bias, out, stats, pool_max, pool_min)
+    if (pool_max is None) != (pool_min is None):
+        raise RuntimeError("monai_amd.conv3d_k3_blk: both pooled tensors or none")
+    if pool_max is not None and (pool_max.shape != pool_min.shape or pool_max.stride() != pool_min.stride() or not pool_max[0].is_contiguous()):
+        raise RuntimeError("monai_amd.conv3d_k3_blk: pool_max / pool_min must be two equally laid out [N, C, D/2, H/2, W/2] tensors, dense per sample")
+    xi, xo = _lib.tensor5(x, x_nrm), _lib.tensor5(out)
+    _lib.lib().call("mh_conv3d_k3_blk_f32", int(cfg), C.byref(xi), int(in_block), _lib.ptr(packed_w), _lib.ptr(bias), C.byref(xo), int(out_block), _lib.ptr(stats),
+                    int(bool(accumulate)), _lib.ptr(pool_max), _lib.ptr(pool_min), 0 if pool_max is None else int(pool_max.stride(0)), _s(x))
+    return out
+
+
+def to_blk16(x: torch.Tensor, out: Optional[torch.Tensor] = None) -> torch.Tensor:
+    n, c, d, h, w = x.shape
+    if c % 16:
+        raise RuntimeError("monai_amd.to_blk16: C must be a multiple of 16")
+    out = torch.empty_like(x, memory_format=torch.contiguous_format) if out is None else out
+    out.as_strided((n, c // 16, d, h, w, 16), (out.stride(0), 16 * d * h * w, 16 * h * w, 16 * w, 16, 1)).copy_(x.reshape(n, c // 16, 16, d, h, w).permute(0, 1, 3, 4, 5, 2))
+    return out
+
+
+def from_blk16(x: torch.Tensor) -> torch.Tensor:
+    n, c, d, h, w = x.shape
+    v = x.as_strided((n, c // 16, d, h, w, 16), (x.stride(0), 16 * d * h * w, 16 * h * w, 16 * w, 16, 1))
+    return v.permute(0, 1, 5, 2, 3, 4).reshape(n, c, d, h, w).contiguous()
 
 
 def pool_select(pool_max: torch.Tensor, pool_min: torch.Tensor, nrm: torch.Tensor) -> torch.Tensor:
```

After: 208.0 million voxels/s (median of 6 runs). About the same (+1.0%).
